# gchq/annchor

Hardware: AMD Instinct MI355X
Metric: knn_graph_builds_per_s (1 / Annchor.fit() wall-clock; BASELINE: k-NN graph build time + recall@k) (higher is better)
Workload: dtype int32 bit-vectors (Levenshtein) + f64 (bounds/regression/selection); 1 GPU; load_strings Levenshtein N=1600 n_anchors=15 k=25 p_work=0.12 niters=2; parallelism=one GPU

## Files before the change

annchor_amd/_native.py:

```python
import ctypes
import os

import numpy as np

_HERE = os.path.dirname(os.path.abspath(__file__))
LIB_PATH = os.environ.get("ANNCHOR_HIP_LIB", os.path.join(_HERE, "libannchor_hip.so"))

F_D, F_A, F_SID, F_IJS, F_I_PTR, F_I_IDX, F_FEATURES, F_NCM, F_RA, F_LABELS, F_THRESH, F_PROB, F_CAND, F_NEXT, F_DAD = range(1, 16)
_FIELD_DTYPE = {
    F_D: np.float64, F_A: np.int64, F_SID: np.uint64, F_IJS: np.int64, F_I_PTR: np.int64, F_I_IDX: np.int64,
    F_FEATURES: np.float64, F_NCM: np.uint8, F_RA: np.float64, F_LABELS: np.int64, F_THRESH: np.float64,
    F_PROB: np.float64, F_CAND: np.int64, F_NEXT: np.int64, F_DAD: np.float64,
}

METRIC_LEVENSHTEIN, METRIC_EUCLIDEAN_F32, METRIC_EUCLIDEAN_F64, METRIC_WASSERSTEIN = 1, 2, 3, 4
METRIC_COSINE_F32, METRIC_COSINE_F64 = 5, 6

_vp, _i32, _i64, _dbl = ctypes.c_void_p, ctypes.c_int32, ctypes.c_int64, ctypes.c_double
_SIGNATURES = {
    "annchor_create": (ctypes.c_int, [ctypes.c_int, ctypes.POINTER(_vp)]),
    "annchor_destroy": (None, [_vp]),
    "annchor_release_parked": (ctypes.c_int, []),
    "annchor_parked_bytes": (ctypes.c_int, [ctypes.c_int, ctypes.POINTER(_i64)]),
    "annchor_last_error": (ctypes.c_char_p, [_vp]),
# ... 7 lines not shown
    "annchor_set_strings": (ctypes.c_int, [_vp, _vp, _vp, _vp, _i64, _i32]),
    "annchor_set_strings_u16": (ctypes.c_int, [_vp, _vp, _vp, _vp, _i64, _i32]),
    "annchor_set_points_f32": (ctypes.c_int, [_vp, _vp, _i64, _i32]),
    "annchor_set_points_f64": (ctypes.c_int, [_vp, _vp, _i64, _i32]),
    "annchor_set_points_cosine_f32": (ctypes.c_int, [_vp, _vp, _i64, _i32]),
    "annchor_set_points_cosine_f64": (ctypes.c_int, [_vp, _vp, _i64, _i32]),
    "annchor_set_histograms": (ctypes.c_int, [_vp, _vp, _i64, _i32, _vp]),
    "annchor_set_opaque": (ctypes.c_int, [_vp, _i64]),
    "annchor_metric_pairs": (ctypes.c_int, [_vp, _vp, _i64, _vp]),
    "annchor_brute_force": (ctypes.c_int, [_vp, _i32, _vp, _vp]),
    "annchor_pick_anchors_maxmin": (ctypes.c_int, [_vp, _i32, _i64]),
    "annchor_pick_anchors_selected": (ctypes.c_int, [_vp, _vp, _i32]),
    "annchor_set_anchor_distances": (ctypes.c_int, [_vp, _vp, _i32, _vp, _i32]),
    "annchor_build_locality": (ctypes.c_int, [_vp, _i32, _i32, _i32, ctypes.POINTER(_i64), ctypes.POINTER(_i64)]),
    "annchor_build_query_locality": (ctypes.c_int, [_vp, _i64, _i32, _i32, ctypes.POINTER(_i64), ctypes.POINTER(_i64)]),
    "annchor_compute_features": (ctypes.c_int, [_vp]),
    "annchor_count_uncomputed": (ctypes.c_int, [_vp, ctypes.POINTER(_i64)]),
    "annchor_kth_uncomputed_dad": (ctypes.c_int, [_vp, _vp, _i32, _vp]),
    "annchor_bin_counts": (ctypes.c_int, [_vp, _vp, _i32, _vp]),
    "annchor_sampler_stats": (ctypes.c_int, [_vp, _vp, _i32, _vp, _vp, _vp, _vp]),
    "annchor_select_by_rank": (ctypes.c_int, [_vp, _vp, _i32, _vp, _vp, _i64, _vp]),
    "annchor_sample_pairs": (ctypes.c_int, [_vp, _vp, _i32, _vp, _vp, _vp, _i64, _vp, _vp, _vp]),
    "annchor_sample_pairs_device": (ctypes.c_int, [_vp, _vp, _i32, _vp, _vp, _vp, _i64]),
    "annchor_hash_sample_pairs_device": (ctypes.c_int, [_vp, _vp, _i32, _vp, _vp, ctypes.c_uint64, _vp]),
    "annchor_download_samples": (ctypes.c_int, [_vp, _vp, _vp, _vp, _vp]),
    "annchor_fit_regression_device": (ctypes.c_int, [_vp, _vp, _i32, _i32, _i32]),
    "annchor_fit_errors_device": (ctypes.c_int, [_vp]),
    "annchor_model_download": (ctypes.c_int, [_vp, _vp, _vp, _vp, _vp, _vp]),
    "annchor_errors_download": (ctypes.c_int, [_vp, _vp, _i64]),
    "annchor_model_download_with_errors": (ctypes.c_int, [_vp, _vp, _vp, _vp, _vp, _vp, _vp, _i64, ctypes.POINTER(_i64)]),
    "annchor_sample_pairs_device_draw": (ctypes.c_int, [_vp, _vp, _i32, _vp, _vp, ctypes.c_uint32, ctypes.POINTER(_i64), ctypes.POINTER(_i32)]),
    "annchor_legacy_choice_ranks_device": (ctypes.c_int, [_vp, ctypes.c_uint32, _vp, _vp, _i32, _vp, ctypes.POINTER(_i32)]),
    "annchor_hash_sample": (ctypes.c_int, [_vp, _vp, _i32, _vp, _vp, ctypes.c_uint64, _vp, ctypes.POINTER(_i64)]),
    "annchor_hash_sample_pairs": (ctypes.c_int, [_vp, _vp, _i32, _vp, _vp, ctypes.c_uint64, _vp, _vp, _vp, ctypes.POINTER(_i64)]),
    "annchor_legacy_prefetch": (ctypes.c_int, [ctypes.c_uint32, _i64]),
    "annchor_legacy_generate": (ctypes.c_int, [ctypes.c_uint32, _i64]),
    "annchor_legacy_generate_at_next_wait": (ctypes.c_int, [_vp, ctypes.c_uint32, _i64, _i64]),
    "annchor_legacy_choice_ranks": (ctypes.c_int, [ctypes.c_uint32, _vp, _vp, _i32, _vp, _vp]),
    "annchor_legacy_choice_begin": (ctypes.c_int, [ctypes.c_uint32, _vp, _vp, _i32, ctypes.POINTER(_vp)]),
    "annchor_legacy_choice_end": (ctypes.c_int, [_vp, _vp, _vp]),
    "annchor_ols_bins": (ctypes.c_int, [_vp, _vp, _vp, _i64, _i32, _vp, _i32, _vp, _vp, _vp, _vp]),
    "annchor_gather_features": (ctypes.c_int, [_vp, _vp, _i64, _vp]),
    "annchor_evaluate_samples": (ctypes.c_int, [_vp, _vp, _i64, _vp]),
    "annchor_set_samples": (ctypes.c_int, [_vp, _vp, _i64, _vp]),
    "annchor_predict_merge": (ctypes.c_int, [_vp, _vp, _i32, _vp, _vp, _i32, _i32, _vp]),
    "annchor_merge_host_prediction": (ctypes.c_int, [_vp, _vp, _i32, _i32]),
    "annchor_set_labels": (ctypes.c_int, [_vp, _vp]),
    "annchor_select_candidates": (ctypes.c_int, [_vp, _i32, _i32, _vp, _vp, _i32, _i64, _i32,
                                                 ctypes.POINTER(_i64), ctypes.POINTER(_i64)]),
    "annchor_select_prepare": (ctypes.c_int, [_vp, _i32, _i32]),
    "annchor_mark_candidates": (ctypes.c_int, [_vp]),
    "annchor_refine_candidates": (ctypes.c_int, [_vp]),
    "annchor_park_refine": (ctypes.c_int, [_vp, _i32]),
    "annchor_set_refined": (ctypes.c_int, [_vp, _vp, _i64]),
    "annchor_update_bounds": (ctypes.c_int, [_vp]),
    "annchor_neighbor_graph": (ctypes.c_int, [_vp, _i32, _vp, _vp]),
    "annchor_stream_bind": (ctypes.c_int, [_vp, _vp, _i64, _i32, _i64, _i32]),
    "annchor_stream_anchor_round": (ctypes.c_int, [_vp, _vp, _i32, _i32, ctypes.POINTER(_dbl), ctypes.POINTER(_i64)]),
    "annchor_stream_get_row": (ctypes.c_int, [_vp, _i64, _vp]),
    "annchor_stream_order": (ctypes.c_int, [_vp, _i32] + [ctypes.POINTER(_vp)] * 6 + [ctypes.POINTER(_i64), ctypes.POINTER(_i32),
                                                                                   ctypes.POINTER(_i32)]),
    "annchor_stream_knn": (ctypes.c_int, [_vp, _vp, _vp, _vp, _vp, _vp, _vp, _i64, _i32, _i32, _i32, _i32, _i32, _i32, _dbl, _i32, _i32, _vp,
                                          _vp, _vp, ctypes.POINTER(_i64)]),
    "annchor_stream_knn_begin": (ctypes.c_int, [_vp, _vp, _vp, _vp, _vp, _vp, _vp, _i64, _i32, _i32, _i32, _i32, _i32, _i32, _i32,
                                                ctypes.POINTER(_vp), ctypes.POINTER(_i64)]),
    "annchor_stream_knn_join": (ctypes.c_int, [_vp, _vp, _i32, ctypes.POINTER(_vp), ctypes.POINTER(_i64)]),
    "annchor_stream_join_rev_begin": (ctypes.c_int, [_vp, _vp, ctypes.POINTER(_vp), ctypes.POINTER(_vp), ctypes.POINTER(_i64)]),
    "annchor_stream_order_begin": (ctypes.c_int, [_vp, _i32, _i32, _i32, ctypes.POINTER(_vp), ctypes.POINTER(_vp), ctypes.POINTER(_i64)]),
    "annchor_stream_order_end": (ctypes.c_int, [_vp] + [ctypes.POINTER(_vp)] * 6 + [ctypes.POINTER(_i64), ctypes.POINTER(_i32),
                                                                                       ctypes.POINTER(_i32)]),
    "annchor_stream_last_counts": (ctypes.c_int, [_vp, ctypes.POINTER(_i64), ctypes.POINTER(_i64)]),
    "annchor_stream_last_kernel": (ctypes.c_int, [_vp, ctypes.POINTER(ctypes.c_int32), ctypes.POINTER(_i64)]),
    "annchor_stream_last_tile_kernels": (ctypes.c_int, [_vp, ctypes.POINTER(ctypes.c_int32), ctypes.POINTER(ctypes.c_int32)]),
    "annchor_stream_budget": (ctypes.c_int, [_i32, _dbl, _i32, ctypes.POINTER(_i32), ctypes.POINTER(_i32), ctypes.POINTER(_i32)]),
    "annchor_stream_knn_end": (ctypes.c_int, [_vp, _vp, _vp, _vp, ctypes.POINTER(_i64)]),
    "annchor_stream_knn_run": (ctypes.c_int, [_vp, _vp, _vp, _vp, _vp, _vp, _vp, _i64, _i32, _i32, _i32, _i32, _i32, _i32, _dbl, _i32, _i32,
                                               ctypes.POINTER(_i64)]),
    "annchor_stream_knn_fetch": (ctypes.c_int, [_vp, _vp, _vp, _vp]),
    "annchor_stream_query": (ctypes.c_int, [_vp, _vp, _vp, _vp, _vp, _vp, _vp, _i64, _i32, _i32, _i32, _i32, _dbl, _vp, _vp,
                                            ctypes.POINTER(_i64)]),
    "annchor_stream_bind_f64": (ctypes.c_int, [_vp, _vp, _i64, _i32, _i64, _vp, _vp, ctypes.POINTER(_vp)]),
    "annchor_stream_rerank64": (ctypes.c_int, [_vp, _i32, _vp, _vp]),
    "annchor_stream_query64": (ctypes.c_int, [_vp, _vp, _vp, _vp, _vp, _vp, _vp, _i64, _i32, _i32, _i32, _i32, _i32, _dbl, _vp, _i64, _i64,
                                              _vp, _vp, ctypes.POINTER(_i64)]),
    "annchor_stream_last_rerank64": (ctypes.c_int, [_vp, ctypes.POINTER(_i64), ctypes.POINTER(ctypes.c_int32)]),
    "annchor_stream_order_classes": (ctypes.c_int, [_vp, _vp, _i32, _vp, ctypes.POINTER(_i64), ctypes.POINTER(_i32), ctypes.POINTER(_i32)]),
    "annchor_stream_enemies": (ctypes.c_int, [_vp, _i32, _dbl, _vp, _vp, ctypes.POINTER(_i64)]),
    "annchor_stream_join_tables": (ctypes.c_int, [_vp, _vp, _i32, _i32, _i32, _vp]),
    "annchor_stream_hip_stream": (ctypes.c_int, [_vp, ctypes.POINTER(_vp)]),
    "annchor_stream_anchor_begin": (ctypes.c_int, [_vp, _i32, _i64, _i32, ctypes.POINTER(_vp), ctypes.POINTER(_vp), ctypes.POINTER(_i64)]),
    "annchor_stream_anchor_step": (ctypes.c_int, [_vp, _vp, _i32, _i32]),
    "annchor_stream_anchor_end": (ctypes.c_int, [_vp, _vp, _vp]),
    "annchor_stream_rows_begin": (ctypes.c_int, [_vp, _i32, _vp, ctypes.POINTER(_vp), ctypes.POINTER(_vp), ctypes.POINTER(_i64)]),
    "annchor_stream_rows_end": (ctypes.c_int, [_vp, _i32, _vp]),
    "annchor_stream_anchor_dists_begin": (ctypes.c_int, [_vp, _i32, _vp, ctypes.POINTER(_vp), ctypes.POINTER(_vp), ctypes.POINTER(_i64)]),
    "annchor_stream_lists_all": (ctypes.c_int, [_vp, _i32, _i64, ctypes.POINTER(_vp)]),
    "annchor_stream_route_begin": (ctypes.c_int, [_vp, _i32, _vp, _vp, ctypes.POINTER(_vp), _vp, ctypes.POINTER(_i64), ctypes.POINTER(_i64)]),
    "annchor_stream_route_recv": (ctypes.c_int, [_vp, _i64, ctypes.POINTER(_vp)]),
    "annchor_comm_unique_id": (ctypes.c_int, [_vp]),
    "annchor_comm_init": (ctypes.c_int, [_vp, _vp, _i32, _i32]),
    "annchor_comm_destroy": (ctypes.c_int, [_vp]),
    "annchor_comm_set_timeout": (ctypes.c_int, [_vp, ctypes.c_double]),
    "annchor_comm_preflight": (ctypes.c_int, [_vp, ctypes.c_double]),
    "annchor_comm_init_side": (ctypes.c_int, [_vp, _vp]),
    "annchor_comm_allgather_begin": (ctypes.c_int, [_vp, _vp, _vp, _i64]),
    "annchor_comm_side_join": (ctypes.c_int, [_vp]),
# ... 491 lines not shown
        pos, y = _c(pos, np.int64), _c(y, np.float64)
        self._chk(self.lib.annchor_set_samples(self.h, _ptr(pos), len(pos), _ptr(y)))

    def predict_merge(self, bins, W, c, first, is_metric, n_samples):
        bins, W, c = _c(bins, np.float64), _c(W, np.float64), _c(c, np.float64)
        sp = np.zeros(n_samples, dtype=np.float64)
        self._chk(self.lib.annchor_predict_merge(self.h, _ptr(bins), len(bins) - 1, _ptr(W), _ptr(c), int(first),
                                                 int(is_metric), _ptr(sp)))
        return sp

    def n_pairs(self):
        return self.field_size(F_NCM)

    def merge_host_prediction(self, pred, first, is_metric):
        pred = _c(pred, np.float64).reshape(-1)
        if pred.shape[0] != self.n_pairs():
            raise ValueError("regression.predict returned %d values for %d candidate pairs" % (pred.shape[0], self.n_pairs()))
        self._chk(self.lib.annchor_merge_host_prediction(self.h, _ptr(pred), int(first), int(is_metric)))

    def set_labels(self, labels):
        labels = _c(labels, np.int64).reshape(-1)
        if labels.shape[0] != self.n_pairs():
            raise ValueError("error_predictor.predict returned %d labels for %d candidate pairs" % (labels.shape[0], self.n_pairs()))
        if labels.size and (labels.min() < 0 or labels.max() >= 255):
            raise ValueError("error labels must lie in 0..254 (got %d..%d)" % (labels.min(), labels.max()))
        self._chk(self.lib.annchor_set_labels(self.h, _ptr(labels)))

    def select_candidates(self, n_neighbors, nmin, errs_list, n_refine, lookahead, n_labels=None):
        nc, nn = _i64(), _i64()
        if errs_list is None:
            self._chk(self.lib.annchor_select_candidates(self.h, int(n_neighbors), int(nmin), None, None, int(n_labels), int(n_refine),
                                                         int(lookahead), ctypes.byref(nc), ctypes.byref(nn)))
            return nc.value, nn.value
        ptr = np.zeros(len(errs_list) + 1, dtype=np.int64)
        np.cumsum([len(e) for e in errs_list], out=ptr[1:])
        errs = _c(np.concatenate(errs_list) if len(errs_list) else np.zeros(0), np.float64)
        self._chk(self.lib.annchor_select_candidates(self.h, int(n_neighbors), int(nmin), _ptr(errs), _ptr(ptr),
                                                     len(errs_list), int(n_refine), int(lookahead),
                                                     ctypes.byref(nc), ctypes.byref(nn)))
        return nc.value, nn.value

    def select_prepare(self, n_neighbors, nmin):
        self._chk(self.lib.annchor_select_prepare(self.h, int(n_neighbors), int(nmin)))

    def mark_candidates(self):
        self._chk(self.lib.annchor_mark_candidates(self.h))

    def refine_candidates(self):
        self._chk(self.lib.annchor_refine_candidates(self.h))

    def park_refine(self, action):
        self._chk(self.lib.annchor_park_refine(self.h, int(action)))

    def set_refined(self, exact):
        exact = _c(exact, np.float64)
        self._chk(self.lib.annchor_set_refined(self.h, _ptr(exact), len(exact)))

    def update_bounds(self):
        self._chk(self.lib.annchor_update_bounds(self.h))

    def neighbor_graph(self, k):
        idx = np.zeros((self.nx, k), dtype=np.int64)
        dist = np.zeros((self.nx, k), dtype=np.float64)
        self._chk(self.lib.annchor_neighbor_graph(self.h, int(k), _ptr(idx), _ptr(dist)))
        return idx, dist

    def stream_bind(self, X, global_base=0, device_ptr=None, shape=None):
        if device_ptr is not None:
            n, d = shape
            self._chk(self.lib.annchor_stream_bind(self.h, device_ptr, int(n), int(d), int(global_base), 1))
        else:
            X = _c(X, np.float32)
            n, d = X.shape
            self._chk(self.lib.annchor_stream_bind(self.h, _ptr(X), n, d, int(global_base), 0))
        self.nx, self.metric = int(n), METRIC_EUCLIDEAN_F32
        self._stream_dim = int(d)

    def stream_bind_f64(self, X, global_base=0, centre=None):
        X = _c(X, np.float64)
        n, d = X.shape
        cin = _c(centre, np.float64) if centre is not None else None
        if cin is not None and cin.shape != (d,):
            raise ValueError("centre must be float64 [%d]" % d)
        cout, rows = np.empty(d, dtype=np.float64), _vp()
        self._chk(self.lib.annchor_stream_bind_f64(self.h, _ptr(X), n, d, int(global_base), _ptr(cin), _ptr(cout), ctypes.byref(rows)))
        self.nx, self.metric = int(n), METRIC_EUCLIDEAN_F32
        self._stream_dim = int(d)
        return cout, rows.value

    def stream_rerank64(self, k, n_local, out=None):
        if out is not None:
            idx, dist = out.take(n_local, k)
        else:
            idx = np.empty((int(n_local), int(k)), dtype=np.int64)
            dist = np.empty((int(n_local), int(k)), dtype=np.float64)
        self._chk(self.lib.annchor_stream_rerank64(self.h, int(k), _ptr(idx), _ptr(dist)))
        return idx, dist

    def stream_query64(self, cols, n_all, nt_all, n_anchors, dim_padded, nn, nn_search, p_work, rows64, n_data, data_base=0):
        idx = np.empty((self.nx, nn), dtype=np.int64)
        dist = np.empty((self.nx, nn), dtype=np.float64)
        ev = _i64()
        self._chk(self.lib.annchor_stream_query64(self.h, cols["Xs"], cols["rs"], cols["perm"], cols["lo"], cols["hi"], cols["mid"],
                                                  int(n_all), int(nt_all), int(n_anchors), int(dim_padded), int(nn), int(nn_search),
                                                  float(p_work), rows64, int(n_data), int(data_base), _ptr(idx), _ptr(dist), ctypes.byref(ev)))
        return idx, dist, ev.value
# ... 338 lines not shown
```

annchor_amd/annchor.py:

```python
import time
from collections import Counter

import os
import sys

import numpy as np

from . import _native
from .distances import DeviceMetric
from .error_predictors import SimpleStratifiedErrorRegression
from .pickers import MaxMinAnchorPicker
from .regressors import SimpleStratifiedLinearRegression
from .samplers import DeviceStratifiedSampler, NothingToSample, SimpleStratifiedSampler
from .utils import get_exact_ijs_, get_function_from_input, test_parallelisation

from .distances import euclidean as distances_euclidean
from .distances import cosine as distances_cosine

_DRAW_OVERLAP = {"worker": True, "defer": "defer"}[os.environ.get("ANNCHOR_DRAW", "defer")]
PAIRLIST_MAX_POINTS = 30000
PAIRLIST_HARD_MAX = None


PAIRLIST_BITMAP_MAX_POINTS = 400000
# ... 378 lines not shown
                return
            self._samples_on_device = False
            if self._device_metric:
                (self.sample_ixs, self.n_samples, self.sample_bins, self.sample_features,
                 self.sample_y) = self.sampler.finish_device(ticket, evaluate=True)
                self._invalidate("ncm")
                self.evals += self.sample_y.shape[0]
                return
            self.sample_ixs, self.n_samples, self.sample_bins = self.sampler.finish_device(ticket)
        else:
            self.sample_ixs, self.n_samples, self.sample_bins = self.sampler.sample(
                self.features, self.feature_names, self.n_samples, self.not_computed_mask, self.random_seed)
        self.sample_ixs = np.asarray(self.sample_ixs, dtype=np.int64)
        self.sample_features = eng.gather_features(self.sample_ixs)
        if self._device_metric:
            self.sample_y = eng.evaluate_samples(self.sample_ixs)
        else:
            self.sample_ijs = self.IJs[self.sample_ixs]
            self.sample_y = np.asarray(self.get_exact_ijs(self.f, self.X, self.sample_ijs), dtype=np.float64)
            eng.set_samples(self.sample_ixs, self.sample_y)
        self._invalidate("ncm")
        self.evals += self.sample_y.shape[0]

    def fit_predict_regression(self):
        self._pair_list_stage("fit_predict_regression")
        self._model_on_device = False
        if self.__dict__.get("_samples_on_device") and self._models_on_device():
            self._engine.fit_regression_device(self.sample_bins, self._first_merge, self.is_metric)
            self._model_on_device, self._predict_on_device, self._fused_labels = True, True, True
            self._first_merge = False
            self._invalidate("RA", "labels")
            return
        self.regression.fit(self.sample_features, self.feature_names, self.sample_y, sample_bins=self.sample_bins)
        model = self.regression.coefficients() if type(self.regression) is SimpleStratifiedLinearRegression else None
        self._fused_labels = False
        if model is not None:
            bins, W, c = model
            self.sample_predict = self._engine.predict_merge(bins, W, c, self._first_merge, self.is_metric,
                                                             len(self.sample_ixs))
            self._fused_labels = (type(self.error_predictor) is SimpleStratifiedErrorRegression
                                  and self.error_predictor.partition_feature_name == "double anchor distance"
                                  and np.array_equal(bins, self.sample_bins))
        else:
            pred = np.asarray(self.regression.predict(self.features, self.feature_names), dtype=np.float64)
            self.sample_predict = pred[self.sample_ixs]
            self._engine.merge_host_prediction(pred, self._first_merge, self.is_metric)
        self._first_merge = False
        self._invalidate("RA", "labels")

    def fit_predict_errors(self):
        self._pair_list_stage("fit_predict_errors")
        if self._pipelined and self._fit_it is not None:
            nn = self.n_neighbors
            self._engine.select_prepare(nn, 3 * nn // 2 if self._fit_it == 0 else 0)
        if self.__dict__.get("_model_on_device"):
            self._engine.fit_errors_device()
            self._invalidate("labels")
            if self._fit_it is not None and self.__dict__.get("_make_stream"):
                self._make_stream(self._fit_it + 1)
            return
        self.error_predictor.fit(self.sample_features, self.feature_names, self.sample_y - self.sample_predict,
                                 sample_bins=self.sample_bins)
        if not self._fused_labels:
            labels = self._label_slots(self.error_predictor.predict(self.features, self.feature_names))
            self._engine.set_labels(labels)
        self._invalidate("labels")

    def _label_slots(self, labels):
        labels = np.asarray(labels)
        keys = list(self.error_predictor.labels)
        if keys == list(range(len(keys))):
            return labels
        order = np.argsort(np.asarray(keys), kind="stable")
        sk = np.asarray(keys)[order]
        at = np.minimum(np.searchsorted(sk, labels), len(sk) - 1)
        if not np.array_equal(sk[at], labels):
            raise ValueError("error_predictor.predict returned a label that is not in error_predictor.labels")
        return order[at]

    def select_refine_candidate_pairs(self, w=0.5, it=0):
        self._pair_list_stage("select_refine_candidate_pairs")
        nn = self.n_neighbors
        n_refine = int((self.p_work * self.N - self.na - self.n_samples) * w) + 1
        n_refine = 0 if n_refine < 0 else n_refine
        nmin = 3 * nn // 2 if it == 0 else 0
        if self.__dict__.get("_model_on_device"):
            nb = len(self.sample_bins) - 1
            ncand, nnext = self._engine.select_candidates(nn, nmin, None, n_refine, self.lookahead, n_labels=nb)
            self._device_model_nb = nb
        else:
            labels = list(self.error_predictor.labels)
            errs = [np.asarray(self.error_predictor.errs[lab], dtype=np.float64) for lab in labels]
            if labels != list(range(len(labels))) and self._fused_labels:
                raise NotImplementedError("the fused label pass numbers the partitions 0..L-1; got labels %r" % (labels[:8],))
            ncand, nnext = self._engine.select_candidates(nn, nmin, errs, n_refine, self.lookahead)
        self.n_refine = n_refine
        self._invalidate("RA", "thresh", "cand", "next")
        if self._pipelined and self._device_metric and ncand and it < self.niters - 1 and self._sampler_on_device():
            self._engine.mark_candidates()
            self._engine.park_refine(1)
            try:
                self._sample_ticket = self.sampler.begin_device(self._engine, self.n_samples, self.random_seed, overlap=_DRAW_OVERLAP,
                                                                **({"device_trace": True} if self._models_on_device() else {}))
            finally:
                self._engine.park_refine(2)
        elif self._device_metric:
            self._engine.refine_candidates()
        elif ncand:
            mapback = self._engine.download(_native.F_CAND)
            exact = np.asarray(self.get_exact_ijs(self.f, self.X, self.IJs[mapback]), dtype=np.float64)
            self._engine.set_refined(exact)
        self.evals += ncand
        self._invalidate("RA", "ncm")

    def _adopt_device_model(self, nb):
        W, c, status, ep, flags, flat = self._engine.model_download_with_errors(nb, 2 * int(self.n_samples) + 16)
        if flags[0] == 3:
            raise _native.NativeError("sample step: the draw's trace kernel gave up waiting for the host's partner stream "
                                      "(ANNCHOR_DRAW_STREAM_TIMEOUT_MS; ANNCHOR_DRAW_STREAM=0 uploads the partners instead)")
        if flags[0] == 1:
            raise _native.NativeError("sample step: a (bin, rank) entry does not exist (stale counts?)")
        if flags[0] or flags[1] or flags[2] or status.any() or flat is None:
            self._device_model_refused = (status.copy(), flags.copy())
            return False
        reg = self.regression
        reg.n_partitions, reg.sample_bins, reg.coef_, reg.intercept_ = nb, self.sample_bins, W, c
        self._device_err_ptr = ep
        ep_ = self.error_predictor
        ep_.partition_bins, ep_.n_partitions, ep_.labels = self.sample_bins, nb, range(nb)
        ep_.errs = {b: flat[ep[b]:ep[b + 1]].copy() for b in range(nb)}
        return True

    @property
    def nextback(self):
        return self._view("next", lambda: self._engine.download(_native.F_NEXT))

    @property
    def mapback(self):
        return self._view("cand", lambda: self._engine.download(_native.F_CAND))

    def update_anchor_points(self, timeout=None, chunk_size=None):
        self._pair_list_stage("update_anchor_points")
        self._engine.update_bounds()
        self._invalidate("features")

    def get_ann(self):
        self._pair_list_stage("get_ann")
        self.neighbor_graph = self._engine.neighbor_graph(self.n_neighbors)

    def fit(self):
        if self._streamed is not None:
            st = self._streamed.fit()
            self.neighbor_graph = st.neighbor_graph
            if self._cosine_streamed:
                self.neighbor_graph = (st.neighbor_graph[0], st.neighbor_graph[1] ** 2 / 2.0)
            self._cache["A"] = st.A
            self.evals, self.timings = st.evals, st.timings
            return self
        origin = time.perf_counter()
        t = self.timings = {}
        legacy_rng = self._sampler_on_device() and type(self.sampler) is SimpleStratifiedSampler
        ndraws = self.N + self.N // 2 + 4096
        seed0 = self.random_seed + getattr(self.sampler, "loop_num", 0)

        def make_stream(it):
            if legacy_rng and it < self.niters:
                s = time.perf_counter()
                _native.legacy_generate(seed0 + it, ndraws)
                t["rng_stream"] = t.get("rng_stream", 0.0) + time.perf_counter() - s

        self._make_stream = make_stream

        def stage(name, fn, *a, **k):
            s = time.perf_counter()
            fn(*a, **k)
            t[name] = t.get(name, 0.0) + time.perf_counter() - s
            if self.verbose:
                print("%40s: %6.3f | %6.3f" % (name, time.perf_counter() - s, time.perf_counter() - origin))

        evals0, loop0, n_samples0 = self.evals, getattr(self.sampler, "loop_num", None), self.n_samples
        self._pipelined = True
        self._device_models_off = False
        try:
            try:
                return self._fit_stages(stage, make_stream, t, origin)
            except _DeviceModelRefused:
                self.evals, self.n_samples = evals0, n_samples0
                if loop0 is not None:
                    self.sampler.loop_num = loop0
                self._first_merge, self._sample_ticket, self._model_on_device = True, None, False
                t.clear()
                ols, self.ols = self.ols, "lapack"
                try:
                    return self._fit_stages(stage, make_stream, t, origin)
                finally:
                    self.ols = ols
        finally:
            self._pipelined, self._fit_it, self._sample_ticket = False, None, None
            self._make_stream = None

    def _fit_stages(self, stage, make_stream, t, origin):
        stage("get_anchors", self.get_anchors)
        legacy_rng = self._sampler_on_device() and type(self.sampler) is SimpleStratifiedSampler
        ndraws = self.N + self.N // 2 + 4096
        seed0 = self.random_seed + getattr(self.sampler, "loop_num", 0)
        fused = self._models_on_device()
        if self._anchors_on_device:
            if legacy_rng:
                self._engine.legacy_generate_at_next_wait(seed0, ndraws)
        elif legacy_rng:
            _native.legacy_prefetch(seed0, ndraws)
        stage("get_locality", self.get_locality)
        stage("get_features", self.get_features)
        niters = self.niters
        for it in range(niters):
            if legacy_rng and not fused and it + 1 < niters:
                _native.legacy_prefetch(seed0 + it + 1, ndraws)
            try:
                stage("get_sample", self.get_sample)
            except NothingToSample as err:
                if it == 0:
                    raise ValueError("Sampler raised NothingToSample on first iteration.") from err
                print("Warning: main loop terminated early with nothing " + "left to sample.")
                break
            stage("fit_predict_regression", self.fit_predict_regression)
            self._fit_it = it
            stage("fit_predict_errors", self.fit_predict_errors)
            self._fit_it = None
            stage("select_refine_candidate_pairs", self.select_refine_candidate_pairs, w=1 / niters, it=it)
            if it < niters - 1:
                stage("update_anchor_points", self.update_anchor_points)
        stage("get_ann", self.get_ann)
        if self.__dict__.get("_model_on_device") and not self._adopt_device_model(self._device_model_nb):
            raise _DeviceModelRefused()
        t["total"] = time.perf_counter() - origin
        return self

    def query(self, Q, nn=15, p_work=0.3, get_exact_query_ijs=None):
        if self._streamed is not None:
            qt = np.float64 if self._float64_streamed else np.float32
            Qs = np.asarray(Q, dtype=qt)
            if self._cosine_streamed:
                Qs = (Qs / np.linalg.norm(Qs.astype(np.float64), axis=1)[:, None]).astype(qt)
            idx, dist = self._streamed.query(Qs, nn=nn, p_work=p_work)
            return (idx, dist ** 2 / 2.0) if self._cosine_streamed else (idx, dist)
        if self.p_work > 1:
            print("Warning: p_work should not exceed 1.  Setting it to 1.")
            self.p_work = 1.0
        nq, nx = len(Q), self.nx
        na = self.n_anchors * nq
        nbf = nq * nx
        limit = ((nq * nn * 3) // 2 - 1 + na) / nbf
# ... 160 lines not shown
```

annchor_amd/csrc/common.h:

```cpp
#pragma once
#include <hip/hip_runtime.h>

#include <cstdint>
#include <cstdio>
#include <cstring>
#include <string>
#include <vector>
#include <chrono>

#include "../../include/annchor_hip.h"

#define ANN_WAVE 64

struct DevBuf {
    void *p = nullptr;
    size_t cap = 0;
    bool in_arena = false;
    template <typename T> T *as() const { return reinterpret_cast<T *>(p); }
};

struct ProfEntry {
    const char *name;
    double ms = 0;
    int64_t launches = 0;
// ... 62 lines not shown
    void *comm_watch = nullptr;

    int na = 0, nA = 0;
    DevBuf Dt;
    DevBuf A;
    DevBuf anchorRank;
    DevBuf runmin, redval, redidx;

    DevBuf sid, cA, thr;
    int sid_nw = 1;
    DevBuf sidl, sidm;
    int sid_L = 0;
    DevBuf Kbits, Kpref;
    DevBuf deg, low, rowstart;
    DevBuf Iptr, Iidx;
    int64_t n = 0;
    DevBuf ij;
    bool have_bitmap = false;
    DevBuf colT, colM;

    DevBuf lb, ub, dad, RA, prob;
    DevBuf anc, ncm, label;
    bool have_features = false, have_RA = false;
    int64_t n_unc = -1;
    int64_t n_unc_after_features = -1;

    DevBuf spos, sy;
    DevBuf draw_J, draw_next, draw_q1;
    DevBuf sfeat, spred;
    DevBuf model;
    DevBuf ols_scratch;
    std::vector<DevBuf *> own_allocs;
    int prof_group_entry = -1;
    bool model_fitted = false;
    bool errs_on_device = false;
    int model_nb = 0;
    DevBuf dev_flags;
    bool dev_flags_clean = false;
    bool gn_err_clean = false;
    bool state_prewarmed = false;
    DevBuf sstats;
    DevBuf hs_key, hs_pos, hs_misc;
    int64_t nsamp = 0;

    DevBuf thresh;
    DevBuf cand, next;
    int64_t ncand = 0, nnext = 0;
    bool cand_marked = false;
    DevBuf gl_val, gl_pos, gl_cnt, gl_ncomp, marked, markcount;
    DevBuf gn_state;
    bool sel_prepared = false;
    int sel_k = 0, sel_nmin = 0;
    bool gn_pending = false;
    int gn_round = 0, gn_L = 0;
    DevBuf sel_hist, sel_state, blk_cnt, blk_off;
    DevBuf sel_pass_state;
    DevBuf tie_lists, tie_hist;
    const void *tie_hist_clean = nullptr;
    DevBuf sel2, sel_bufA, sel_bufB, sel_seg;
    const void *sel2_clean = nullptr;
    DevBuf errs, errptr;
    DevBuf ecdf_index;
    DevBuf cptr, cidx, cval;
    DevBuf c16, cbnd;
    DevBuf tmp0, tmp1, tmp2, tmp3;
    DevBuf scan_tmp;

    DevBuf stage_in, stage_out;

    bool prof_on = false;
    int prof_mode = 0;
    std::vector<hipEvent_t> ev_pool;
    std::vector<ProfEntry> prof;
    std::vector<PendingEvent> pending;
    hipEvent_t call_a = nullptr, call_b = nullptr;
    bool call_timed = false;
    static constexpr int PIN_SLOTS = 8;
    static constexpr size_t PIN_SLOT_BYTES = 64 * 1024;
    static constexpr size_t PIN_DL_BYTES = 1024 * 1024;
    static constexpr size_t PIN_TAIL_BYTES = 64;
    unsigned char *pin = nullptr;
    hipEvent_t pin_ev[PIN_SLOTS] = {};
    bool pin_busy[PIN_SLOTS] = {};
    int pin_next = 0;
};

const char *ann_set_err(annchor_ctx *c, const char *fmt, ...);

#define ANN_CHECK_HIP(c, expr)                                                                  \
    do {                                                                                        \
        hipError_t _e = (expr);                                                                 \
        if (_e != hipSuccess) {                                                                 \
            ann_set_err((c), "%s:%d: %s failed: %s", __FILE__, __LINE__, #expr,                 \
                        hipGetErrorString(_e));                                                 \
            return ANNCHOR_EHIP;                                                                \
        }                                                                                       \
    } while (0)

#define ANN_TRY(expr)                \
    do {                             \
        int _r = (expr);             \
        if (_r != ANNCHOR_OK) return _r; \
    } while (0)

#define ANN_REQUIRE(c, cond, code, ...)    \
    do {                                   \
        if (!(cond)) {                     \
// ... 37 lines not shown
    ProfScope(annchor_ctx *ctx, const char *name, double alg_bytes = 0);
    ~ProfScope();
};

static inline int ann_blocks(int64_t n, int per_block) { return (int)((n + per_block - 1) / per_block); }

__device__ __forceinline__ uint64_t ann_key_asc(double v)
{
    uint64_t u = (uint64_t)__double_as_longlong(v);
    return (u & 0x8000000000000000ull) ? ~u : (u | 0x8000000000000000ull);
}
__device__ __forceinline__ double ann_key_asc_inv(uint64_t k)
{
    uint64_t u = (k & 0x8000000000000000ull) ? (k & 0x7fffffffffffffffull) : ~k;
    return __longlong_as_double((long long)u);
}

template <typename T> __device__ __forceinline__ T ann_ldc(const T *__restrict__ p, int64_t t, int64_t n)
{
    return p[t < n ? t : n - 1];
}

#define ANN_STREAM_MIN_PAIRS (8ll << 20)
template <typename T> __device__ __forceinline__ void ann_store(T *p, T v, bool stream)
{
    if (stream) __builtin_nontemporal_store(v, p);
    else *p = v;
}
template <typename T> __device__ __forceinline__ T ann_load(const T *p, bool stream)
{
    return stream ? __builtin_nontemporal_load(p) : *p;
}

#define MAXBINS 64
struct RegModel {
    double e[MAXBINS + 1];
    double w[MAXBINS][3];
    double c[MAXBINS];
    int nb;
};
struct DeviceModel {
    RegModel reg;
    int32_t status[MAXBINS];
    int32_t err_status;
    int64_t rows[MAXBINS];
    int64_t errptr[MAXBINS + 1];
};

struct PairSource {
    const int2 *ij = nullptr;
    const int32_t *idx = nullptr;
    const int32_t *anchor = nullptr;
    int64_t n = 0;
    const double *pick_row = nullptr;
    double *pick_runmin = nullptr;
    int32_t *pick_out = nullptr;
    int pick_reset = 0;
    bool *pick_fused = nullptr;
};

#define ANN_MASK_ANCHORS 256
#define ANN_MAX_ANCHORS 1024
static_assert(ANN_MAX_ANCHORS < 0xffff, "wide sets list anchor ids as uint16, 0xffff pads");
static inline bool ann_sid_wide(int na) { return na > ANN_MASK_ANCHORS; }
__device__ __forceinline__ int sidm_common(const uint16_t *__restrict__ sidl, const uint64_t *__restrict__ sidm, int L, int na, int kw,
                                           int64_t i, int64_t w)
{
    const int lane = threadIdx.x & 63;
    int c = 0;
    for (int r = 0; r < L; ++r) {
        const int64_t e = i * L + r;
        const uint32_t pr = reinterpret_cast<const uint32_t *>(sidl)[e >> 1];
        const int a = __builtin_amdgcn_readfirstlane((int)((pr >> ((e & 1) * 16)) & 0xffffu));
        if (a >= na) continue;
        const uint64_t m = sidm[(size_t)a * kw + w];
        c += (int)((m >> lane) & 1ull);
    }
    return c;
}
template <int LC>
__device__ __forceinline__ int sidm_common_l(const uint16_t *__restrict__ sidl, const uint64_t *__restrict__ sidm, int na, int kw,
                                             int64_t i, int64_t w)
{
    const int lane = threadIdx.x & 63;
    int a[LC];
#pragma unroll
    for (int r = 0; r < LC; ++r) {
        const int64_t e = i * LC + r;
        const uint32_t pr = reinterpret_cast<const uint32_t *>(sidl)[e >> 1];
        a[r] = __builtin_amdgcn_readfirstlane((int)((pr >> ((e & 1) * 16)) & 0xffffu));
    }
    int c = 0;
#pragma unroll
    for (int r = 0; r < LC; ++r) {
        const uint64_t m = sidm[(size_t)(a[r] < na ? a[r] : 0) * kw + w];
        c += a[r] < na ? (int)((m >> lane) & 1ull) : 0;
    }
    return c;
}
template <int NW> struct Sid { uint64_t w[NW]; };
template <int NW> __device__ __forceinline__ Sid<NW> sid_ld(const uint64_t *__restrict__ sid, int64_t i)
{
    Sid<NW> s;
#pragma unroll
    for (int w = 0; w < NW; ++w) s.w[w] = sid[i * NW + w];
    return s;
// ... 46 lines not shown
```

annchor_amd/csrc/ctx.hip:

```cpp
#include <cstdarg>
#include <cstdlib>

#include "common.h"
#include <algorithm>
#include <chrono>
#include <mutex>

static std::string g_create_err;
void ann_stream_release(annchor_ctx *c);
void ann_enemies_release(annchor_ctx *c);
void ann_comm_release(annchor_ctx *c);
hipError_t ann_comm_guarded_sync(annchor_ctx *c, hipStream_t stream, const char *where);

const char *ann_set_err(annchor_ctx *c, const char *fmt, ...)
{
    char buf[1024];
    va_list ap;
    va_start(ap, fmt);
    vsnprintf(buf, sizeof buf, fmt, ap);
    va_end(ap);
    if (c && c->comm_aborted && c->err.rfind("collective timed out", 0) == 0) return c->err.c_str();
    if (c) c->err = buf; else g_create_err = buf;
    return c ? c->err.c_str() : g_create_err.c_str();
}
// ... 143 lines not shown
    Piece pieces[] = {{&c->dev_flags, sizeof(int32_t) * 16}, {&c->lev_cursors, 4 * sizeof(int32_t)}, {&c->sel_state, ann_sel_state_bytes()},
                      {&c->sel2, ann_sel2_table_bytes()},    {&c->tie_hist, ann_tie_hist_bytes()},   {&c->lev_ap, slot_bytes}};
    size_t need = 0;
    for (auto &q : pieces) {
        if (q.b->p) return ANNCHOR_OK;
        need += (q.bytes + 255) & ~(size_t)255;
    }
    if (c->arena_off + need > c->arena_size) return ANNCHOR_OK;
    char *first = c->arena + c->arena_off;
    for (auto &q : pieces) ANN_TRY(ann_reserve(c, *q.b, q.bytes));
    ANN_CHECK_HIP(c, hipMemsetAsync(first, 0, need, c->stream));
    c->dev_flags_clean = true;
    c->lev_cursor_epoch = 0;
    c->gn_err_clean = true;
    c->sel2_clean = c->sel2.p;
    c->tie_hist_clean = c->tie_hist.p;
    c->lev_ap_epoch = 0;
    c->state_prewarmed = true;
    return ANNCHOR_OK;
}

int ann_h2d(annchor_ctx *c, void *dst, const void *src, size_t bytes)
{
    if (bytes == 0) return ANNCHOR_OK;
    if (c->pin && bytes <= annchor_ctx::PIN_SLOT_BYTES) {
        const int sl = c->pin_next;
        c->pin_next = (sl + 1) % annchor_ctx::PIN_SLOTS;
        if (c->pin_busy[sl]) ANN_CHECK_HIP(c, hipEventSynchronize(c->pin_ev[sl]));
        unsigned char *slot = c->pin + (size_t)sl * annchor_ctx::PIN_SLOT_BYTES;
        memcpy(slot, src, bytes);
        ANN_CHECK_HIP(c, hipMemcpyAsync(dst, slot, bytes, hipMemcpyHostToDevice, c->stream));
        ANN_CHECK_HIP(c, hipEventRecord(c->pin_ev[sl], c->stream));
        c->pin_busy[sl] = true;
        return ANNCHOR_OK;
    }
    ANN_CHECK_HIP(c, hipMemcpyAsync(dst, src, bytes, hipMemcpyHostToDevice, c->stream));
    ANN_CHECK_HIP(c, ann_sync(c, __func__));
    return ANNCHOR_OK;
}

hipError_t ann_sync(annchor_ctx *c, const char *where)
{
    static const bool trace = getenv("ANNCHOR_SYNC_TRACE") != nullptr;
    static const bool timing = getenv("ANNCHOR_SYNC_TIMING") != nullptr;
    if (trace) fprintf(stderr, "sync %s\n", where);
    const long long t_in = timing ? ann_now_ns() : 0;
    if (c->idle_gen_n > c->idle_gen_done) {
        c->idle_gen_done = std::min(c->idle_gen_n, c->idle_gen_done + c->idle_gen_chunk);
        (void)ann_legacy_generate_upto(c->idle_gen_seed, c->idle_gen_n, c->idle_gen_done);
    }
    const long long t_w = timing ? ann_now_ns() : 0;
    const hipError_t rc = c->comm ? ann_comm_guarded_sync(c, c->stream, where) : hipStreamSynchronize(c->stream);
    if (timing) fprintf(stderr, "T wait %s %lld %lld %lld\n", where, t_in, t_w, ann_now_ns());
    if (c->lev_ap_probe_epoch) ann_lev_ap_probe(c);
    return rc;
}

extern "C" int annchor_legacy_generate_at_next_wait(annchor_ctx *c, uint32_t seed, int64_t ndraws, int64_t chunk)
{
    if (!c || ndraws < 0) return ANNCHOR_EINVAL;
    c->idle_gen_seed = seed;
    c->idle_gen_n = ndraws;
    c->idle_gen_done = 0;
    c->idle_gen_chunk = chunk > 0 ? chunk : ndraws;
    return ANNCHOR_OK;
}

int ann_d2h(annchor_ctx *c, void *dst, const void *src, size_t bytes)
{
    if (bytes == 0) return ANNCHOR_OK;
    if (c->pin && bytes <= annchor_ctx::PIN_DL_BYTES) {
        unsigned char *slot = c->pin + (size_t)annchor_ctx::PIN_SLOTS * annchor_ctx::PIN_SLOT_BYTES;
        ANN_CHECK_HIP(c, hipMemcpyAsync(slot, src, bytes, hipMemcpyDeviceToHost, c->stream));
        ANN_CHECK_HIP(c, ann_sync(c, __func__));
        memcpy(dst, slot, bytes);
        return ANNCHOR_OK;
    }
    ANN_CHECK_HIP(c, hipMemcpyAsync(dst, src, bytes, hipMemcpyDeviceToHost, c->stream));
    ANN_CHECK_HIP(c, ann_sync(c, __func__));
    return ANNCHOR_OK;
}

int ann_d2h2(annchor_ctx *c, void *dst1, const void *src1, size_t bytes1, void *dst2, const void *src2, size_t bytes2)
{
    const size_t off2 = (bytes1 + 63) & ~(size_t)63;
    if (c->pin && off2 + bytes2 <= annchor_ctx::PIN_DL_BYTES) {
        unsigned char *slot = c->pin + (size_t)annchor_ctx::PIN_SLOTS * annchor_ctx::PIN_SLOT_BYTES;
        ANN_CHECK_HIP(c, hipMemcpyAsync(slot, src1, bytes1, hipMemcpyDeviceToHost, c->stream));
        ANN_CHECK_HIP(c, hipMemcpyAsync(slot + off2, src2, bytes2, hipMemcpyDeviceToHost, c->stream));
        ANN_CHECK_HIP(c, ann_sync(c, __func__));
        memcpy(dst1, slot, bytes1);
        memcpy(dst2, slot + off2, bytes2);
        return ANNCHOR_OK;
    }
    ANN_TRY(ann_d2h(c, dst1, src1, bytes1));
    return ann_d2h(c, dst2, src2, bytes2);
}

int ann_d2h_then(annchor_ctx *c, void *dst, const void *src, size_t bytes, int (*then)(annchor_ctx *))
{
    if (!c->pin || bytes > annchor_ctx::PIN_DL_BYTES) {
        ANN_TRY(ann_d2h(c, dst, src, bytes));
        return then(c);
    }
    if (!c->dl_ev) ANN_CHECK_HIP(c, hipEventCreate(&c->dl_ev));
    unsigned char *slot = c->pin + (size_t)annchor_ctx::PIN_SLOTS * annchor_ctx::PIN_SLOT_BYTES;
    ANN_CHECK_HIP(c, hipMemcpyAsync(slot, src, bytes, hipMemcpyDeviceToHost, c->stream));
    ANN_CHECK_HIP(c, hipEventRecord(c->dl_ev, c->stream));
    const int rc = then(c);
    static const bool trace = getenv("ANNCHOR_SYNC_TRACE") != nullptr;
    static const bool timing = getenv("ANNCHOR_SYNC_TIMING") != nullptr;
    if (trace) fprintf(stderr, "sync %s\n", __func__);
    const long long t_w = timing ? ann_now_ns() : 0;
    ANN_CHECK_HIP(c, hipEventSynchronize(c->dl_ev));
    if (timing) fprintf(stderr, "T wait %s %lld %lld %lld\n", __func__, t_w, t_w, ann_now_ns());
    memcpy(dst, slot, bytes);
    return rc;
}

int ann_prof_entry(annchor_ctx *c, const char *name)
{
    for (size_t i = 0; i < c->prof.size(); ++i)
        if (c->prof[i].name == name || strcmp(c->prof[i].name, name) == 0) return (int)i;
    ProfEntry e;
    e.name = name;
    c->prof.push_back(e);
    return (int)c->prof.size() - 1;
}

static void prof_drain(annchor_ctx *c)
{
    for (auto &p : c->pending) {
        float ms = 0;
        if (hipEventSynchronize(p.b) == hipSuccess && hipEventElapsedTime(&ms, p.a, p.b) == hipSuccess)
            c->prof[p.entry].ms += ms;
        c->ev_pool.push_back(p.a);
        c->ev_pool.push_back(p.b);
    }
    c->pending.clear();
}

ProfScope::ProfScope(annchor_ctx *ctx, const char *name, double alg_bytes) : c(ctx)
{
    if (!c->prof_on) return;
    if (c->prof_mode == 2) {
        const size_t n = strlen(name);
        if (n < 6 || strcmp(name + n - 6, "_pairs") != 0) return;
    }
    entry = ann_prof_entry(c, name);
    c->prof[entry].launches += 1;
    c->prof[entry].alg_bytes += alg_bytes;
    if (entry == c->prof_group_entry) { entry = -1; return; }
    auto get = [&](hipEvent_t *e) {
        if (!c->ev_pool.empty()) { *e = c->ev_pool.back(); c->ev_pool.pop_back(); return true; }
        return hipEventCreate(e) == hipSuccess;
    };
    if (!get(&a) || !get(&b)) { entry = -1; return; }
    (void)hipEventRecord(a, c->stream);
}

ProfGroup::ProfGroup(annchor_ctx *ctx, const char *name) : c(ctx)
{
    if (!c->prof_on || c->prof_group_entry >= 0) return;
    if (c->prof_mode == 2) {
        const size_t n = strlen(name);
        if (n < 6 || strcmp(name + n - 6, "_pairs") != 0) return;
    }
// ... 542 lines not shown
```

annchor_amd/csrc/lev.hip:

```cpp
#include <cstdlib>

#include "common.h"
#include <atomic>
#include <type_traits>

#define LEV_THREADS 256
#define LEV_WAVES (LEV_THREADS / ANN_WAVE)

__device__ __forceinline__ uint32_t dpp_wave_shr1(uint32_t v)
{
    return (uint32_t)__builtin_amdgcn_update_dpp((int)v, (int)v, 0x138 , 0xf, 0xf, false);
}

struct LevArgs {
    const uint8_t *sym;
    const int32_t *soff;
    const int32_t *slen;
    const int2 *ij;
    const int32_t *idx;
    const int32_t *anchor;
    int64_t n;
    double *out;
    double *RA;
    uint8_t *ncm;
    int G;
    int P;
    int alphabet;
    int text_stride;
    int pm_bytes;
    int wave_bytes;
};

__device__ __forceinline__ void wave_lds_fence()
{
    __builtin_amdgcn_fence(__ATOMIC_RELEASE, "workgroup");
    __builtin_amdgcn_wave_barrier();
    __builtin_amdgcn_fence(__ATOMIC_ACQUIRE, "workgroup");
}

struct LevArgsR {
    LevArgs b;
    int GL;
    int pm_stride;
    const double *pick_row;
    double *pick_runmin;
    int32_t *pick_out;
    int pick_reset, pick_nx;
    const int32_t *perm;
    const int32_t *n0;
    int GL0, P0;
};

#define LEVR_PAD 64

template <int R> __global__ __launch_bounds__(ANN_WAVE) void k_lev_r(LevArgsR ar)
{
    extern __shared__ __attribute__((aligned(16))) unsigned char smem[];
    const LevArgs &a = ar.b;
    const int lane = threadIdx.x;
    const int GL = ar.GL, P = a.P, A = a.alphabet, PS = ar.pm_stride;
    const int g = lane / GL;
    const int w = lane - g * GL;
    const bool slot_ok = g < P;
    uint32_t *pm_g = reinterpret_cast<uint32_t *>(smem) + (size_t)(slot_ok ? g : 0) * A * PS;
    uint16_t *txt_g = reinterpret_cast<uint16_t *>(smem + a.pm_bytes + (size_t)(slot_ok ? g : 0) * a.text_stride);
    int *ssum = reinterpret_cast<int *>(smem + a.pm_bytes + (size_t)P * a.text_stride);
    const int64_t n_tasks = (a.n + P - 1) / P;
    const uint32_t row_bytes = (uint32_t)PS * 4u;
    typedef uint32_t vecR __attribute__((ext_vector_type(R)));

    if (slot_ok)
        for (int e = w * 8; e < a.text_stride / 2; e += GL * 8) *reinterpret_cast<uint4 *>(txt_g + e) = make_uint4(0, 0, 0, 0);

    int picked = -1;
    if (ar.pick_row) {
        double bv = -INFINITY;
        int bi = 0x7fffffff;
        const int nx = ar.pick_nx;
        for (int j0 = 0; j0 < nx; j0 += 64 * 8) {
            double d[8], rm[8];
#pragma unroll
            for (int e = 0; e < 8; ++e) {
                const int j = min(j0 + e * 64 + lane, nx - 1);
                d[e] = ar.pick_row[j];
                rm[e] = ar.pick_reset ? 0.0 : ar.pick_runmin[j];
            }
#pragma unroll
            for (int e = 0; e < 8; ++e) {
                const int j = j0 + e * 64 + lane;
                if (j < nx) {
                    const double v = ar.pick_reset ? d[e] : fmin(rm[e], d[e]);
                    if (blockIdx.x == 0) ar.pick_runmin[j] = v;
                    argmax_combine(bv, bi, v, j);
                }
            }
        }
#pragma unroll
        for (int off = 32; off > 0; off >>= 1) {
            const double ov = __shfl_xor(bv, off);
            const int oi = __shfl_xor(bi, off);
            argmax_combine(bv, bi, ov, oi);
        }
        picked = bi;
// ... 93 lines not shown
                const uint32_t nvp = hns | ~(d0 | hps), nvn = hps & d0;
                vp[r] = valid ? nvp : vp[r];
                vn[r] = valid ? nvn : vn[r];
                hp_up = hp;
                hn_up = hn;
            }
            out_hp = hp_up;
            out_hn = hn_up;
            __builtin_amdgcn_sched_barrier(0);
            eq = eq_n;
            c1 = c2;
        };
        int k_lo = min(GL - 1, max_steps), k_hi = (active && m > 0) ? n : 0x7fffffff;
#pragma unroll
        for (int off = 32; off > 0; off >>= 1) k_hi = min(k_hi, __shfl_xor(k_hi, off));
        k_hi = max(k_lo, min(__builtin_amdgcn_readfirstlane(k_hi), max_steps));
        int k = 0;
        for (; k < k_lo; ++k) column(k, std::true_type());
        for (; k + 2 <= k_hi; k += 2) { column(k, std::false_type()); column(k + 1, std::false_type()); }
        for (; k < k_hi; ++k) column(k, std::false_type());
        for (; k < max_steps; ++k) column(k, std::true_type());
        if (active) {
            int part = 0;
#pragma unroll
            for (int r = 0; r < R; ++r) {
                const int wi = w * R + r;
                const uint32_t rows = wi < Wp - 1 ? 0xffffffffu : (wi == Wp - 1 ? (0xffffffffu >> (31 - ((m - 1) & 31))) : 0u);
                part += __popc(vp[r] & rows) - __popc(vn[r] & rows);
            }
            if (part) atomicAdd(&ssum[g], part);
        }
        wave_lds_fence();
        if (active && w == 0) {
            const double d = (double)(n + ssum[g]);
            if (a.out) a.out[t_pair] = d;
            if (a.RA) { a.RA[opos] = d; a.ncm[opos] = 0; }
        }
        wave_lds_fence();
    }
}

template <int R> static int launch_r(annchor_ctx *c, LevArgs a, int64_t npairs, const PairSource &src)
{
    const int W = (c->maxlen + 31) / 32 > 0 ? (c->maxlen + 31) / 32 : 1;
    LevArgsR ar;
    ar.GL = (W + R - 1) / R;
    ar.pm_stride = ar.GL * R;
    a.G = ar.GL;
    a.P = 64 / ar.GL;
    a.pm_bytes = (int)((((size_t)a.P * a.alphabet * ar.pm_stride * 4) + 15) & ~(size_t)15);
    a.text_stride = 2 * (2 * LEVR_PAD + ((c->maxlen + 15) & ~15) + 16);
    a.wave_bytes = a.pm_bytes + a.P * a.text_stride + 256;
    ar.b = a;
    ar.pick_row = nullptr; ar.pick_runmin = nullptr; ar.pick_out = nullptr; ar.pick_reset = 0; ar.pick_nx = 0;
    if (src.anchor && src.pick_fused && c->nx <= 8192) {
        *src.pick_fused = true;
        if (src.pick_row) {
            ar.pick_row = src.pick_row; ar.pick_runmin = src.pick_runmin; ar.pick_out = src.pick_out;
            ar.pick_reset = src.pick_reset; ar.pick_nx = (int)c->nx;
        }
    }
    const size_t lds = (size_t)a.wave_bytes;
    ANN_REQUIRE(c, lds <= 160 * 1024, ANNCHOR_ELIMIT, "alphabet %d x length %d needs %zu B of LDS (> 160 KiB)", c->alphabet,
                c->maxlen, lds);
    if (lds > 64 * 1024)
        ANN_CHECK_HIP(c, hipFuncSetAttribute((const void *)k_lev_r<R>, hipFuncAttributeMaxDynamicSharedMemorySize, (int)lds));
    int64_t blocks = (npairs + a.P - 1) / a.P;
    const int64_t max_blocks = (int64_t)c->prop.multiProcessorCount * 32;
    if (blocks > max_blocks) blocks = max_blocks;
    k_lev_r<R><<<(int)blocks, ANN_WAVE, lds, c->stream>>>(ar);
    ANN_CHECK_HIP(c, hipGetLastError());
    return ANNCHOR_OK;
}


__device__ __forceinline__ uint32_t dpp_shr1_or(uint32_t v, uint32_t m)
{
    return (uint32_t)__builtin_amdgcn_update_dpp(0, (int)v, 0x138, 0xf, 0xf, true) | m;
}
__device__ __forceinline__ uint32_t dpp_shr1_and(uint32_t v, uint32_t m)
{
    return (uint32_t)__builtin_amdgcn_update_dpp(0, (int)v, 0x138, 0xf, 0xf, true) & m;
}

#define LEVF_ROW 128

__global__ __launch_bounds__(ANN_WAVE) void k_lev_f(LevArgsR ar)
{
    extern __shared__ __attribute__((aligned(16))) unsigned char smem[];
    const LevArgs &a = ar.b;
    const int lane = threadIdx.x;
    const int A = a.alphabet;
    unsigned char *pm_col = smem + (size_t)(lane >> 5) * A * LEVF_ROW + (size_t)(lane & 31) * 4;
    const int Pmax = ar.perm ? ar.P0 : a.P;
    int *ssum = reinterpret_cast<int *>(smem + a.pm_bytes + (size_t)Pmax * a.text_stride);

    int picked = -1;
    if (ar.pick_row) {
        double bv = -INFINITY;
        int bi = 0x7fffffff;
        const int nx = ar.pick_nx;
        for (int j0 = 0; j0 < nx; j0 += 64 * 8) {
            double d[8], rm[8];
#pragma unroll
            for (int e = 0; e < 8; ++e) {
                const int j = min(j0 + e * 64 + lane, nx - 1);
                d[e] = ar.pick_row[j];
                rm[e] = ar.pick_reset ? 0.0 : ar.pick_runmin[j];
            }
#pragma unroll
            for (int e = 0; e < 8; ++e) {
                const int j = j0 + e * 64 + lane;
                if (j < nx) {
                    const double v = ar.pick_reset ? d[e] : fmin(rm[e], d[e]);
                    if (blockIdx.x == 0) ar.pick_runmin[j] = v;
                    argmax_combine(bv, bi, v, j);
                }
            }
        }
#pragma unroll
        for (int off = 32; off > 0; off >>= 1) {
            const double ov = __shfl_xor(bv, off);
            const int oi = __shfl_xor(bi, off);
            argmax_combine(bv, bi, ov, oi);
        }
        picked = bi;
        if (blockIdx.x == 0 && lane == 0) *ar.pick_out = bi;
    }
    const int64_t n_short = ar.perm ? (int64_t)*ar.n0 : 0;
  for (int cls = ar.perm ? 0 : 1; cls < 2; ++cls) {
    const int GL = cls == 0 ? ar.GL0 : ar.GL, P = cls == 0 ? ar.P0 : a.P;
    const int64_t n_cls = ar.perm ? (cls == 0 ? n_short : a.n - n_short) : a.n;
    const int g = lane / GL;
    const int w = lane - g * GL;
    const bool slot_ok = g < P;
    uint8_t *txt_g = smem + a.pm_bytes + (size_t)(slot_ok ? g : 0) * a.text_stride;
    const int64_t n_tasks = (n_cls + P - 1) / P;
    if (slot_ok)
        for (int e = w * 16; e < a.text_stride; e += GL * 16) *reinterpret_cast<uint4 *>(txt_g + e) = make_uint4(0, 0, 0, 0);
    uint32_t hp_or = w == 0 ? 0x80000000u : 0u;
    uint32_t hn_and = w == 0 ? 0u : 0xffffffffu;
    asm volatile("" : "+v"(hp_or), "+v"(hn_and));

// ... 54 lines not shown
            const uint32_t c2 = tp[k + 2];
            const uint32_t eq_n = *reinterpret_cast<const uint32_t *>(pm_col + c1 * LEVF_ROW);
            const uint32_t hp_up = dpp_shr1_or(out_hp, hp_or), hn_up = dpp_shr1_and(out_hn, hn_and);
            __builtin_amdgcn_sched_barrier(0);
            const bool valid = !decltype(checked)::value || (uint32_t)(k - w) < un;
            const uint32_t c = hn_up >> 31;
            const uint32_t x = eq | c;
            const uint32_t t = __builtin_amdgcn_bitop3_b32(c, eq, vp, 0xa8);
            const uint32_t sm = t + vp;
            const uint32_t d0p = __builtin_amdgcn_bitop3_b32(sm, vp, x, 0xbe);
            const uint32_t hp = __builtin_amdgcn_bitop3_b32(vn, d0p, vp, 0xf1);
            const uint32_t d0 = d0p | vn;
            const uint32_t hn = d0 & vp;
            const uint32_t hps = __builtin_amdgcn_alignbit(hp, hp_up, 31);
            const uint32_t hns = __builtin_amdgcn_alignbit(hn, hn_up, 31);
            const uint32_t nvp = __builtin_amdgcn_bitop3_b32(hns, d0, hps, 0xf1);
            const uint32_t nvn = hps & d0;
            vp = valid ? nvp : vp;
            vn = valid ? nvn : vn;
            out_hp = hp;
            out_hn = hn;
            __builtin_amdgcn_sched_barrier(0);
            eq = eq_n;
            c1 = c2;
        };
        int k_lo = min(GL - 1, max_steps), k_hi = (active && m > 0) ? n : 0x7fffffff;
#pragma unroll
        for (int off = 32; off > 0; off >>= 1) k_hi = min(k_hi, __shfl_xor(k_hi, off));
        k_hi = max(k_lo, min(__builtin_amdgcn_readfirstlane(k_hi), max_steps));
        int k = 0;
        for (; k < k_lo; ++k) column(k, std::true_type());
        for (; k + 2 <= k_hi; k += 2) { column(k, std::false_type()); column(k + 1, std::false_type()); }
        for (; k < k_hi; ++k) column(k, std::false_type());
        for (; k < max_steps; ++k) column(k, std::true_type());
        if (active) {
            const uint32_t rows = w < Wp - 1 ? 0xffffffffu : (w == Wp - 1 ? (0xffffffffu >> (31 - ((m - 1) & 31))) : 0u);
            const int part = __popc(vp & rows) - __popc(vn & rows);
            if (part) atomicAdd(&ssum[g], part);
        }
        wave_lds_fence();
        if (active && w == 0) {
            const double d = (double)(n + ssum[g]);
            if (a.out) a.out[t_pair] = d;
            if (a.RA) { a.RA[opos] = d; a.ncm[opos] = 0; }
        }
        wave_lds_fence();
    }
  }
}

__global__ __launch_bounds__(256) void k_lev_classify(const int2 *__restrict__ ij, const int32_t *__restrict__ idx,
                                                      const int32_t *__restrict__ slen, int64_t n, int gl0,
                                                      int32_t *__restrict__ perm, int32_t *__restrict__ cursors,
                                                      int32_t *__restrict__ next_cursors)
{
    if (blockIdx.x == 0 && threadIdx.x < 2) next_cursors[threadIdx.x] = 0;
    __shared__ int wcnt[2][4];
    __shared__ int base[2];
    const int lane = threadIdx.x & 63, wave = threadIdx.x >> 6;
    const int64_t t = (int64_t)blockIdx.x * 256 + threadIdx.x;
    bool is_short = false, is_long = false;
    if (t < n) {
        const int2 p = ij[idx ? idx[t] : t];
        const int m = min(slen[p.x], slen[p.y]);
        is_short = ((m + 31) >> 5) <= gl0;
        is_long = !is_short;
    }
    const unsigned long long bs = __ballot(is_short), bl = __ballot(is_long);
    if (lane == 0) { wcnt[0][wave] = __popcll(bs); wcnt[1][wave] = __popcll(bl); }
    __syncthreads();
    if (threadIdx.x < 2) {
        const int tot = wcnt[threadIdx.x][0] + wcnt[threadIdx.x][1] + wcnt[threadIdx.x][2] + wcnt[threadIdx.x][3];
        base[threadIdx.x] = tot ? atomicAdd(&cursors[threadIdx.x], tot) : 0;
    }
    __syncthreads();
    const unsigned long long below = (1ull << lane) - 1ull;
    if (is_short) {
        int r = base[0] + __popcll(bs & below);
        for (int q = 0; q < wave; ++q) r += wcnt[0][q];
        perm[r] = (int32_t)t;
    } else if (is_long) {
        int r = base[1] + __popcll(bl & below);
        for (int q = 0; q < wave; ++q) r += wcnt[1][q];
        perm[n - 1 - r] = (int32_t)t;
    }
}

static int lev_next_cursors(annchor_ctx *c, int32_t **cur, int32_t **nxt)
{
    if (!c->lev_cursors.p) {
        ANN_TRY(ann_reserve(c, c->lev_cursors, 4 * sizeof(int32_t)));
        ANN_CHECK_HIP(c, hipMemsetAsync(c->lev_cursors.p, 0, 4 * sizeof(int32_t), c->stream));
        c->lev_cursor_epoch = 0;
    }
    *cur = c->lev_cursors.as<int32_t>() + 2 * (c->lev_cursor_epoch & 1);
    *nxt = c->lev_cursors.as<int32_t>() + 2 * ((c->lev_cursor_epoch + 1) & 1);
    ++c->lev_cursor_epoch;
    return ANNCHOR_OK;
}

static int launch_f(annchor_ctx *c, LevArgs a, int64_t npairs, const PairSource &src)
{
    const int W = (c->maxlen + 31) / 32 > 0 ? (c->maxlen + 31) / 32 : 1;
    LevArgsR ar;
    ar.GL = W;
    ar.pm_stride = 32;
    a.G = ar.GL;
    a.P = 64 / ar.GL;
    a.pm_bytes = 2 * a.alphabet * LEVF_ROW;
    a.text_stride = 2 * LEVR_PAD + ((c->maxlen + 15) & ~15) + 16;
    ar.perm = nullptr; ar.n0 = nullptr; ar.GL0 = 0; ar.P0 = 0;
    static const int cls_min = getenv("ANNCHOR_LEV_CLASS_MIN") ? atoi(getenv("ANNCHOR_LEV_CLASS_MIN")) : 4096;
    if (!src.anchor && c->lev_gl0 > 0 && npairs >= cls_min && npairs < (1ll << 31)) {
        const double fp = 1.0 - (1.0 - c->lev_frac0) * (1.0 - c->lev_frac0);
        const int P0 = 64 / c->lev_gl0;
        const double cost = fp * (double)a.P / (double)P0 + (1.0 - fp);
        if (cost < 0.93) {
            ANN_TRY(ann_reserve(c, c->lev_perm, sizeof(int32_t) * ((size_t)npairs + 4)));
            int32_t *perm = c->lev_perm.as<int32_t>();
            int32_t *cursors = nullptr, *next_cursors = nullptr;
            ANN_TRY(lev_next_cursors(c, &cursors, &next_cursors));
            k_lev_classify<<<ann_blocks(npairs, 256), 256, 0, c->stream>>>(src.ij, src.idx, a.slen, npairs, c->lev_gl0, perm,
                                                                           cursors, next_cursors);
            ar.perm = perm; ar.n0 = cursors; ar.GL0 = c->lev_gl0; ar.P0 = P0;
        }
    }
    a.wave_bytes = a.pm_bytes + (ar.perm ? ar.P0 : a.P) * a.text_stride + 256;
    ar.b = a;
    ar.pick_row = nullptr; ar.pick_runmin = nullptr; ar.pick_out = nullptr; ar.pick_reset = 0; ar.pick_nx = 0;
    if (src.anchor && src.pick_fused && c->nx <= 8192) {
        *src.pick_fused = true;
        if (src.pick_row) {
            ar.pick_row = src.pick_row; ar.pick_runmin = src.pick_runmin; ar.pick_out = src.pick_out;
            ar.pick_reset = src.pick_reset; ar.pick_nx = (int)c->nx;
        }
    }
    const size_t lds = (size_t)a.wave_bytes;
    ANN_REQUIRE(c, lds <= 160 * 1024, ANNCHOR_ELIMIT, "alphabet %d x length %d needs %zu B of LDS (> 160 KiB)", c->alphabet,
                c->maxlen, lds);
    if (lds > 64 * 1024)
        ANN_CHECK_HIP(c, hipFuncSetAttribute((const void *)k_lev_f, hipFuncAttributeMaxDynamicSharedMemorySize, (int)lds));
    int64_t blocks = (npairs + a.P - 1) / a.P;
    const int64_t max_blocks = (int64_t)c->prop.multiProcessorCount * 32;
    if (blocks > max_blocks) blocks = max_blocks;
    k_lev_f<<<(int)blocks, ANN_WAVE, lds, c->stream>>>(ar);
    ANN_CHECK_HIP(c, hipGetLastError());
    return ANNCHOR_OK;
}

struct LevArgsA {
    const uint8_t *sym;
    const int32_t *soff;
    const int32_t *slen;
    const int32_t *anchor;
    int64_t n;
    double *out;
    int alphabet, text_stride, pm_bytes, fb_stride;
    const double *pick_row;
    double *pick_runmin;
    int32_t *pick_out;
    int pick_reset, pick_nx;
};

struct LevArgsA2 {
    LevArgsA a;
    const int32_t *order;
    int n_short;
    int buf_stride;
    int pad;
};

__global__ __launch_bounds__(ANN_WAVE) void k_lev_a2(LevArgsA2 aa)
{
    extern __shared__ __attribute__((aligned(16))) unsigned char smem[];
    const LevArgsA &a = aa.a;
    const int lane = threadIdx.x, A = a.alphabet;
    const int ws = (aa.n_short + 1) >> 1;
    const bool packed = (int)blockIdx.x < ws;
    const int GL = packed ? 16 : 32;
    const int slot = lane / GL, w = lane - slot * GL, pair = slot >> 1, half = slot & 1;
    const int LP = packed ? 32 : 64;
// ... 134 lines not shown
        out_hn = hn;
        __builtin_amdgcn_sched_barrier(0);
        eq = eq_n;
        c1 = c2;
    };
    int k = 0;
    for (; k < k_lo; ++k) column(k, std::true_type());
    for (; k + 2 <= k_hi; k += 2) { column(k, std::false_type()); column(k + 1, std::false_type()); }
    for (; k < k_hi; ++k) column(k, std::false_type());
    for (; k < max_steps; ++k) column(k, std::true_type());

    const uint32_t rows = !have ? 0u : (w < Wp - 1 ? 0xffffffffu : (w == Wp - 1 ? (0xffffffffu >> (31 - ((m - 1) & 31))) : 0u));
    const int part = __popc(vp & rows) - __popc(vn & rows);
    int incl = part;
#pragma unroll
    for (int off = 1; off < 32; off <<= 1) {
        const int o = __shfl_up(incl, off, 32);
        if (w >= off) incl += o;
    }
    int val = (int)un + incl - part;
    if (m == 0) val = half ? n - h : h;
    int16_t *fbp = FB + (size_t)(pair < 2 ? pair : 0) * 2 * a.fb_stride;
    int16_t *fb = fbp + (size_t)half * a.fb_stride;
    if (have && w == 0) fb[0] = (int16_t)val;
#pragma unroll
    for (int b = 0; b < 32; ++b) {
        val += (int)((vp >> b) & 1u) - (int)((vn >> b) & 1u);
        if ((rows >> b) & 1u) fb[w * 32 + b + 1] = (int16_t)val;
    }
    wave_lds_fence();
    int best = 0x7fffffff;
    const int lp = lane & (LP - 1);
    if (have)
        for (int i = lp; i <= m; i += LP) best = min(best, (int)fbp[i] + (int)fbp[a.fb_stride + m - i]);
#pragma unroll
    for (int off = 32; off > 0; off >>= 1)
        if (off < LP) best = min(best, __shfl_xor(best, off));
    if (have && lp == 0) a.out[tq[pair]] = (double)best;
}

struct LevArgsP2 {
    const uint8_t *sym;
    const int32_t *soff;
    const int32_t *slen;
    const int2 *ij;
    const int32_t *idx;
    const int32_t *perm;
    const int32_t *cursors;
    int64_t n;
    double *out;
    double *RA;
    uint8_t *ncm;
    int alphabet, pm_bytes, fb_stride, buf_stride, pad;
};

__global__ __launch_bounds__(ANN_WAVE) void k_lev_p2(LevArgsP2 aa)
{
    extern __shared__ __attribute__((aligned(16))) unsigned char smem[];
    const LevArgsP2 &a = aa;
    const int lane = threadIdx.x, A = a.alphabet;
    const int n_short = a.cursors[0], n_long = a.cursors[1];
    const int ws = (n_short + 1) >> 1;
    for (int task = blockIdx.x; task < ws + n_long; task += gridDim.x) {
    const bool packed = task < ws;
    const int GL = packed ? 16 : 32;
    const int slot = lane / GL, w = lane - slot * GL, pair = slot >> 1, half = slot & 1;
    const int LP = packed ? 32 : 64;
    unsigned char *pm_col = smem + (size_t)(lane >> 5) * A * LEVF_ROW + (size_t)(lane & 31) * 4;
    uint8_t *bufs = smem + a.pm_bytes;
    int16_t *FB = reinterpret_cast<int16_t *>(bufs + 4 * aa.buf_stride);
    for (int e = lane * 16; e < 4 * aa.buf_stride; e += 64 * 16) *reinterpret_cast<uint4 *>(bufs + e) = make_uint4(0, 0, 0, 0);
    uint32_t hp_or = w == 0 ? 0x80000000u : 0u;
    uint32_t hn_and = w == 0 ? 0u : 0xffffffffu;
    asm volatile("" : "+v"(hp_or), "+v"(hn_and));
    int tq[2] = {-1, -1};
    if (packed) {
        tq[0] = a.perm[2 * task];
        if (2 * task + 1 < n_short) tq[1] = a.perm[2 * task + 1];
    } else {
        tq[0] = a.perm[n_short + (task - ws)];
    }
    int si[2] = {0, 0}, sj[2] = {0, 0}, li[2] = {0, 0}, lj[2] = {0, 0};
    int64_t opos[2] = {0, 0};
#pragma unroll
    for (int q = 0; q < 2; ++q)
        if (tq[q] >= 0) {
            opos[q] = a.idx ? (int64_t)a.idx[tq[q]] : (int64_t)tq[q];
            const int2 pq = a.ij[opos[q]];
            si[q] = pq.x; sj[q] = pq.y;
        }
#pragma unroll
    for (int q = 0; q < 2; ++q)
        if (tq[q] >= 0) {
            li[q] = a.slen[si[q]]; lj[q] = a.slen[sj[q]];
            const uint8_t *s0 = a.sym + a.soff[si[q]], *s1 = a.sym + a.soff[sj[q]];
            for (int ch = lane; ch < ((li[q] + 15) >> 4); ch += 64)
                reinterpret_cast<uint4 *>(bufs + (2 * q) * aa.buf_stride + aa.pad)[ch] = reinterpret_cast<const uint4 *>(s0)[ch];
            for (int ch = lane; ch < ((lj[q] + 15) >> 4); ch += 64)
                reinterpret_cast<uint4 *>(bufs + (2 * q + 1) * aa.buf_stride + aa.pad)[ch] = reinterpret_cast<const uint4 *>(s1)[ch];
        }
    wave_lds_fence();
    const bool have = pair < 2 && tq[pair < 2 ? pair : 0] >= 0 && (packed || pair == 0);
    const int pq = pair < 2 ? pair : 0;
    const int l0 = have ? li[pq] : 0, l1 = have ? lj[pq] : 0;
    const bool first_is_pattern = packed ? (l0 <= l1) : (l0 > l1);
    const int m = have ? (first_is_pattern ? l0 : l1) : 0;
    const int n = have ? (first_is_pattern ? l1 : l0) : 0;
    const uint8_t *pat = bufs + (2 * pq + (first_is_pattern ? 0 : 1)) * aa.buf_stride + aa.pad;
    const uint8_t *txt = bufs + (2 * pq + (first_is_pattern ? 1 : 0)) * aa.buf_stride + aa.pad;
    const int Wp = (m + 31) >> 5;
    for (int c = 0; c < A; ++c) *reinterpret_cast<uint32_t *>(pm_col + (size_t)c * LEVF_ROW) = 0u;
    if (have && w < Wp) {
// ... 350 lines not shown
            bool collected = (int)blockIdx.x >= ngroups;
            int polls = 0;
            for (;;) {
                if (!collected) {
                    const unsigned long long v = __hip_atomic_load(sl + min((int)blockIdx.x * 64 + lane, a.ntasks - 1), __ATOMIC_RELAXED,
                                                                   __HIP_MEMORY_SCOPE_AGENT);
                    if (__all((uint32_t)(v >> 32) == tag)) {
                        uint32_t gm = (uint32_t)v;
#pragma unroll
                        for (int off = 32; off > 0; off >>= 1) gm = max(gm, (uint32_t)__shfl_xor((int)gm, off));
                        if (lane == 0)
                            __hip_atomic_store(pl + blockIdx.x, ((unsigned long long)tag << 32) | gm, __ATOMIC_RELAXED, __HIP_MEMORY_SCOPE_AGENT);
                        collected = true;
                    }
                }
                if (collected) {
                    const unsigned long long v = __hip_atomic_load(pl + min(lane, ngroups - 1), __ATOMIC_RELAXED, __HIP_MEMORY_SCOPE_AGENT);
                    mx = (uint32_t)v;
                    if (__all((uint32_t)(v >> 32) == tag)) break;
                }
                if ((++polls & 7) == 0 || a.timeout_ticks == 0) {
                    if (__hip_atomic_load(a.abort_epoch, __ATOMIC_RELAXED, __HIP_MEMORY_SCOPE_AGENT) == a.epoch) return;
                    if (wall_clock64() - t0 > a.timeout_ticks) {
                        if (lane == 0) __hip_atomic_store(a.abort_epoch, a.epoch, __ATOMIC_RELAXED, __HIP_MEMORY_SCOPE_AGENT);
                        return;
                    }
                }
            }
#pragma unroll
            for (int off = 32; off > 0; off >>= 1) mx = max(mx, (uint32_t)__shfl_xor((int)mx, off));
            si = 0xffff - (int)(mx & 0xffffu);
            AP_STAMP(6);
        }
    }
    if (RESCUE) {
        __syncthreads();
        for (int j = threadIdx.x; j < nx; j += blockDim.x) a.rank[j] = -1;
        __syncthreads();
        if (threadIdx.x == 0)
            for (int r = 0; r < a.na; ++r) a.rank[s_A[r]] = r;
    } else {
        if (lane == 0) {
            a.rank[tq0] = rk0;
            if (tq1 >= 0) a.rank[tq1] = rk1;
        }
    }
}

static int launch_p2(annchor_ctx *c, const PairSource &src, double *d_out, double *d_RA, uint8_t *d_ncm)
{
    LevArgsP2 a;
    a.sym = c->sym.as<uint8_t>(); a.soff = c->soff.as<int32_t>(); a.slen = c->slen.as<int32_t>();
    a.ij = src.ij; a.idx = src.idx; a.n = src.n; a.out = d_out; a.RA = d_RA; a.ncm = d_ncm;
    a.alphabet = c->alphabet;
    a.pm_bytes = 2 * a.alphabet * LEVF_ROW;
    a.fb_stride = (c->maxlen + 2 + 7) & ~7;
    a.pad = ((c->maxlen / 2 + 48) + 15) & ~15;
    a.buf_stride = 2 * a.pad + ((c->maxlen + 15) & ~15) + 16;
    const size_t lds = (size_t)a.pm_bytes + 4 * (size_t)a.buf_stride + 4 * sizeof(int16_t) * a.fb_stride;
    ANN_REQUIRE(c, lds <= 160 * 1024, ANNCHOR_ELIMIT, "alphabet %d x length %d needs %zu B of LDS (> 160 KiB)", c->alphabet,
                c->maxlen, lds);
    ANN_TRY(ann_reserve(c, c->lev_perm, sizeof(int32_t) * (size_t)(src.n + 2)));
    int32_t *perm = c->lev_perm.as<int32_t>();
    int32_t *cursors = nullptr, *next_cursors = nullptr;
    ANN_TRY(lev_next_cursors(c, &cursors, &next_cursors));
    k_lev_classify<<<ann_blocks(src.n, 256), 256, 0, c->stream>>>(src.ij, src.idx, a.slen, src.n, 16, perm, cursors, next_cursors);
    a.perm = perm; a.cursors = cursors;
    if (lds > 64 * 1024)
        ANN_CHECK_HIP(c, hipFuncSetAttribute((const void *)k_lev_p2, hipFuncAttributeMaxDynamicSharedMemorySize, (int)lds));
    const int64_t L = c->nx - c->lev_nshort;
    const int64_t long_bound = std::min<int64_t>(src.n, L * (L + 1) / 2);
    const int64_t grid = std::min<int64_t>(src.n, (src.n + 1) / 2 + long_bound + 8);
    k_lev_p2<<<(int)grid, ANN_WAVE, lds, c->stream>>>(a);
    ANN_CHECK_HIP(c, hipGetLastError());
    return ANNCHOR_OK;
}

static int launch_a2(annchor_ctx *c, const PairSource &src, double *d_out)
{
    LevArgsA2 aa;
    LevArgsA &a = aa.a;
    a.sym = c->sym.as<uint8_t>(); a.soff = c->soff.as<int32_t>(); a.slen = c->slen.as<int32_t>();
    a.anchor = src.anchor; a.n = src.n; a.out = d_out; a.alphabet = c->alphabet;
    a.pm_bytes = 2 * a.alphabet * LEVF_ROW;
    a.text_stride = 2 * LEVR_PAD + ((c->maxlen + 15) & ~15) + 16;
    a.fb_stride = (c->maxlen + 2 + 7) & ~7;
    a.pick_row = nullptr; a.pick_runmin = nullptr; a.pick_out = nullptr; a.pick_reset = 0; a.pick_nx = 0;
    if (src.pick_fused && c->nx <= 8192) {
        *src.pick_fused = true;
        if (src.pick_row) {
            a.pick_row = src.pick_row; a.pick_runmin = src.pick_runmin; a.pick_out = src.pick_out;
            a.pick_reset = src.pick_reset; a.pick_nx = (int)c->nx;
        }
    }
    aa.order = c->lev_order.as<int32_t>();
    aa.n_short = c->lev_nshort;
    aa.pad = ((c->maxlen / 2 + 48) + 15) & ~15;
    aa.buf_stride = 2 * aa.pad + ((c->maxlen + 15) & ~15) + 16;
    size_t lds = (size_t)a.pm_bytes + 3 * (size_t)aa.buf_stride + 4 * sizeof(int16_t) * a.fb_stride;
    ANN_REQUIRE(c, lds <= 160 * 1024, ANNCHOR_ELIMIT, "alphabet %d x length %d needs %zu B of LDS (> 160 KiB)", c->alphabet,
                c->maxlen, lds);
    const int64_t blocks = (c->lev_nshort + 1) / 2 + (c->nx - c->lev_nshort);
    {
        const char *e = getenv("ANNCHOR_LEV_A2_LDS");
        const size_t want = e ? (size_t)atoll(e) : (size_t)40 * 1024;
        if (blocks <= (int64_t)c->prop.multiProcessorCount * 4 && want > lds && want <= 160 * 1024) lds = want;
    }
    if (lds > 64 * 1024)
        ANN_CHECK_HIP(c, hipFuncSetAttribute((const void *)k_lev_a2, hipFuncAttributeMaxDynamicSharedMemorySize, (int)lds));
    k_lev_a2<<<(int)blocks, ANN_WAVE, lds, c->stream>>>(aa);
    ANN_CHECK_HIP(c, hipGetLastError());
    return ANNCHOR_OK;
}

static std::atomic<int> g_lev_ap_strikes{0};
static std::atomic<int> g_lev_ap_off{0};
void ann_lev_ap_probe(annchor_ctx *c)
{
    const uint32_t epoch = c->lev_ap_probe_epoch;
// ... 211 lines not shown
            const uint32_t cin = hn_up >> 31;
            const uint32_t x = eq | cin;
            const uint32_t d0 = (((x & vp) + vp) ^ vp) | x | vn;
            const uint32_t hp = vn | ~(d0 | vp);
            const uint32_t hn = d0 & vp;
            const uint32_t hps = __builtin_amdgcn_alignbit(hp, hp_up, 31);
            const uint32_t hns = __builtin_amdgcn_alignbit(hn, hn_up, 31);
            const uint32_t nvp = hns | ~(d0 | hps), nvn = hps & d0;
            vp = valid ? nvp : vp;
            vn = valid ? nvn : vn;
            out_hp = hp;
            out_hn = hn;
        }
        if (active) {
            const uint32_t rows = w < Wp - 1 ? 0xffffffffu : (w == Wp - 1 ? (0xffffffffu >> (31 - ((m - 1) & 31))) : 0u);
            const int part = __popc(vp & rows) - __popc(vn & rows);
            if (part) atomicAdd(&ssum[g], part);
        }
        wave_lds_fence();
        if (active && w == 0) {
            const double d = (double)(n + ssum[g]);
            if (a.out) a.out[t_pair] = d;
            if (a.RA) { a.RA[opos] = d; a.ncm[opos] = 0; }
        }
        wave_lds_fence();
    }
}

static int launch_w(annchor_ctx *c, const PairSource &src, double *d_out, double *d_RA, uint8_t *d_ncm)
{
    LevArgsW a;
    a.sym = c->sym.as<uint16_t>(); a.soff = c->soff.as<int32_t>(); a.slen = c->slen.as<int32_t>();
    a.ij = src.ij; a.idx = src.idx; a.anchor = src.anchor; a.n = src.n; a.out = d_out; a.RA = d_RA; a.ncm = d_ncm;
    const int W = std::max(1, (c->maxlen + 31) / 32);
    ANN_REQUIRE(c, W <= 64, ANNCHOR_ELIMIT, "strings longer than 2048 symbols are not supported by this build (max %d)", c->maxlen);
    a.GL = W; a.P = 64 / W;
    a.text_stride = 2 * LEVR_PAD + ((c->maxlen + 7) & ~7) + 8;
    const size_t lds = (size_t)a.P * a.text_stride * 2 + 256;
    ANN_REQUIRE(c, lds <= 160 * 1024, ANNCHOR_ELIMIT, "strings of %d symbols need %zu B of LDS", c->maxlen, lds);
    if (lds > 64 * 1024)
        ANN_CHECK_HIP(c, hipFuncSetAttribute((const void *)k_lev_w, hipFuncAttributeMaxDynamicSharedMemorySize, (int)lds));
    int64_t blocks = (src.n + a.P - 1) / a.P;
    const int64_t max_blocks = (int64_t)c->prop.multiProcessorCount * 32;
    if (blocks > max_blocks) blocks = max_blocks;
    ProfScope ps(c, "levenshtein_pairs", (double)src.n * (4.0 * c->maxlen + 8));
    k_lev_w<<<(int)blocks, ANN_WAVE, lds, c->stream>>>(a);
    ANN_CHECK_HIP(c, hipGetLastError());
    return ANNCHOR_OK;
}

int ann_lev_launch(annchor_ctx *c, const PairSource &src, double *d_out, double *d_RA, uint8_t *d_ncm)
{
    if (src.n == 0) return ANNCHOR_OK;
    if (c->sym_wide) return launch_w(c, src, d_out, d_RA, d_ncm);
    LevArgs a;
    a.sym = c->sym.as<uint8_t>();
    a.soff = c->soff.as<int32_t>();
    a.slen = c->slen.as<int32_t>();
    a.ij = src.ij;
    a.idx = src.idx;
    a.anchor = src.anchor;
    a.n = src.n;
    a.out = d_out;
    a.RA = d_RA;
    a.ncm = d_ncm;
    int G = (c->maxlen + 31) / 32;
    if (G < 1) G = 1;
    ANN_REQUIRE(c, G <= 64, ANNCHOR_ELIMIT, "strings longer than 2048 symbols are not supported by this build (max %d)",
                c->maxlen);
    a.G = G;
    a.P = 64 / G;
    a.alphabet = c->alphabet;
    a.text_stride = ((c->maxlen + 15) & ~15) + 16;
    a.pm_bytes = (int)((((size_t)a.P * a.alphabet * G * 4) + 15) & ~(size_t)15);
    a.wave_bytes = a.pm_bytes + a.P * a.text_stride + 256;
    const char *env_r = getenv("ANNCHOR_LEV_R");
    {
        const int W = (c->maxlen + 31) / 32;
        const int R = env_r && atoi(env_r) == 1 ? 1 : 9;
        const char *env_a = getenv("ANNCHOR_LEV_ANCHOR");
        const bool anchor_split = !(env_a && atoi(env_a) == 0);
        if (src.anchor && d_out && !d_RA && R == 9 && W <= 32 && anchor_split && c->maxlen < 32000) {
            if (src.n == c->nx && c->lev_order.p) {
                ProfScope ps(c, "levenshtein_pairs", (double)src.n * (2.0 * c->maxlen + 8));
                return launch_a2(c, src, d_out);
            }
        }
        if (R == 9 && W <= 32) {
            ProfScope ps(c, "levenshtein_pairs", (double)src.n * (2.0 * c->maxlen + 8));
            const char *env_p = getenv("ANNCHOR_LEV_P2_MAX");
            const int pf = c->lev_gl0 > 0 ? std::max(1, 64 / c->lev_gl0) : a.P;
            const double cap = (double)c->prop.multiProcessorCount * 4.0 * pf;
            const bool p2 = env_p ? src.n <= atoll(env_p)
                                  : (pf <= 4 && ((double)src.n <= 0.37 * cap || ((double)src.n > cap && (double)src.n <= 1.83 * cap)));
            if (!src.anchor && src.ij && p2 && src.n >= 64 && c->maxlen < 32000) return launch_p2(c, src, d_out, d_RA, d_ncm);
            return launch_f(c, a, src.n, src);
        }
        ProfScope ps(c, "levenshtein_pairs", (double)src.n * (2.0 * c->maxlen + 8));
        return launch_r<1>(c, a, src.n, src);
    }
}
```

annchor_amd/csrc/select.hip:

```cpp
#include "common.h"
#include "rowsel.h"
#include "selstate.h"

__global__ __launch_bounds__(ROW_THREADS) void k_row_thresh(const int64_t *__restrict__ Iptr, RowSrc src, uint32_t k,
                                                           double *__restrict__ thresh, int cap)
{
    __shared__ RowSelShared sh;
    __shared__ RowCand rc;
    extern __shared__ __attribute__((aligned(16))) unsigned char dyn_rt[];
    uint64_t *keys = reinterpret_cast<uint64_t *>(dyn_rt);
    const int64_t i = row_of_block(gridDim.x);
    const int64_t b = Iptr[i];
    const int len = (int)(Iptr[i + 1] - b);
    if (len <= 0) { if (threadIdx.x == 0) thresh[i] = -INFINITY; return; }
    const RowView rv = row_view(src, i, b);
    const uint32_t kk = k >= (uint32_t)len ? (uint32_t)len - 1 : k;
    {
        const int cnt = row_candidates(rc, len, (int)kk + 1, [&](int s) { return ann_key_asc(rv.val(s)); }, [](int) { return true; },
                                       [](int, uint64_t, bool) {});
        const int cnts = cnt > (int)kk ? row_cand_shrink(rc, cnt, (int)kk + 1, src.shrink_min) : -1;
        if (cnts > (int)kk) {
            for (int e = threadIdx.x; e < cnts; e += ROW_THREADS) {
                const uint64_t ke = rc.key[e];
                uint32_t less = 0, leq = 0;
// ... 76 lines not shown
        if (kk < t) {
            const uint32_t o = atomicAdd(&cnt_lt, 1u);
            lkey[o] = kk; lslot[o] = s;
        }
    }
    __syncthreads();
    const uint32_t nlt = cnt_lt;
    uint32_t run = nlt;
    for (int base = 0; base < len && run < (uint32_t)want; base += ROW_THREADS) {
        const int s = base + threadIdx.x;
        const uint32_t f = (s < len && kf(s) == t) ? 1u : 0u;
        uint32_t tot;
        const uint32_t ex = row_block_scan(f, sh.wsum, &tot);
        if (f && run + ex < (uint32_t)want) { lkey[run + ex] = t; lslot[run + ex] = s; }
        run += tot;
        __syncthreads();
    }
    __syncthreads();
    for (int e = threadIdx.x; e < want; e += ROW_THREADS) {
        const uint64_t ke = lkey[e];
        const int32_t se = lslot[e];
        int r = 0;
        for (int o = 0; o < want; ++o) r += (lkey[o] < ke) || (lkey[o] == ke && lslot[o] < se);
        const int32_t p = Iidx[b + se];
        const int2 q = ij[p];
        gl_val[i * L + r] = ann_key_asc_inv(ke);
        gl_pos[i * L + r] = p;
        gl_oth[i * L + r] = q.x == (int)i ? q.y : q.x;
    }
}

__global__ void k_gn_twin(int64_t nx, int L, const int32_t *__restrict__ gl_pos, const int32_t *__restrict__ gl_oth,
                          const int32_t *__restrict__ gl_cnt, int32_t *__restrict__ gl_twin)
{
    const int64_t t = (int64_t)blockIdx.x * blockDim.x + threadIdx.x;
    if (t >= nx * L) return;
    const int64_t i = t / L;
    const int e = (int)(t - i * L);
    int tw = -1;
    if (e < gl_cnt[i]) {
        const int32_t p = gl_pos[t], j = gl_oth[t];
        const int cj = gl_cnt[j];
        for (int o = 0; o < cj; ++o)
            if (gl_pos[(int64_t)j * L + o] == p) { tw = o; break; }
    }
    gl_twin[t] = tw;
}

__global__ __launch_bounds__(256) void k_gn_round(int64_t nx, int nmin, int L, int Lw, const double *__restrict__ gl_val,
                                                 const int32_t *__restrict__ gl_oth, const int32_t *__restrict__ gl_twin,
                                                 const int32_t *__restrict__ gl_cnt, const int32_t *__restrict__ gl_ncomp,
                                                 const uint32_t *__restrict__ cur, uint32_t *__restrict__ nxt,
                                                 const int32_t *__restrict__ mout_cur, int32_t *__restrict__ mout_nxt,
                                                 int32_t *__restrict__ mout_clr, int32_t *__restrict__ changed, int32_t *__restrict__ err)
{
    const int lane = threadIdx.x & 63;
    const int64_t i = ((int64_t)blockIdx.x * blockDim.x + threadIdx.x) >> 6;
    if (i >= nx) return;
    if (lane == 0) mout_clr[i] = 0;
    const int cnt = gl_cnt[i], ncomp = gl_ncomp[i];
    const int ntodo = nmin - ncomp;
    const int chunks = (L + 63) / 64;
    bool active = !(ntodo <= 0 || (cnt == 0 && ncomp == 0));
    if (active && cnt <= ntodo && cnt < L) { if (lane == 0) *err = 1; active = false; }
    int m = active ? mout_cur[i] : 0;
    if (active)
        for (int ch = 0; ch < chunks; ++ch) {
            const int e = ch * 64 + lane;
            bool earlier = false;
            if (e < cnt) {
                const int32_t o = gl_oth[i * L + e], tw = gl_twin[i * L + e];
                earlier = o < i && tw >= 0 && ((cur[(int64_t)o * Lw + (tw >> 5)] >> (tw & 31)) & 1u);
            }
            m += __popcll(__ballot(earlier));
        }
    const int need = ntodo + 1 - m;
    double t = 0;
    bool found = false;
    if (active && need > 0) {
        int cum = 0;
        for (int ch = 0; ch < chunks && !found; ++ch) {
            const int e = ch * 64 + lane;
            bool um = false;
            double v = 0.0;
            if (e < cnt) {
                const int32_t o = gl_oth[i * L + e], tw = gl_twin[i * L + e];
                v = gl_val[i * L + e];
                um = !(o < i && tw >= 0 && ((cur[(int64_t)o * Lw + (tw >> 5)] >> (tw & 31)) & 1u));
            }
            const unsigned long long mb = __ballot(um);
            const int cm = __popcll(mb);
            if (cum + cm >= need) {
                const int want = need - cum - 1;
                const int myrank = __popcll(mb & ((1ull << lane) - 1ull));
                const unsigned long long hit = __ballot(um && myrank == want);
                t = __shfl(v, __ffsll((unsigned long long)hit) - 1);
                found = true;
            }
            cum += cm;
        }
        if (!found && lane == 0) *err = 2;
    }
    bool diff = false;
    for (int ch = 0; ch < chunks; ++ch) {
        const int e = ch * 64 + lane;
        bool mark = false;
        int32_t o = 0, tw = -1;
        if (found && e < cnt) {
            o = gl_oth[i * L + e]; tw = gl_twin[i * L + e];
            const bool earlier = o < i && tw >= 0 && ((cur[(int64_t)o * Lw + (tw >> 5)] >> (tw & 31)) & 1u);
            mark = !earlier && gl_val[i * L + e] < t;
        }
        const unsigned long long mb = __ballot(mark);
        const int w0 = 2 * ch, w1 = 2 * ch + 1;
        if (lane == 0) {
            if (w0 < Lw) { const uint32_t v0 = (uint32_t)mb; diff |= cur[i * Lw + w0] != v0; nxt[i * Lw + w0] = v0; }
            if (w1 < Lw) { const uint32_t v1 = (uint32_t)(mb >> 32); diff |= cur[i * Lw + w1] != v1; nxt[i * Lw + w1] = v1; }
        }
        if (mark && tw < 0 && o > i) atomicAdd(&mout_nxt[o], 1);
    }
    if (lane == 0 && diff) atomicOr(changed, 1);
}

__global__ void k_gn_apply(int64_t nx, int L, int Lw, const int32_t *__restrict__ gl_pos, const int32_t *__restrict__ gl_cnt,
                           const uint32_t *__restrict__ masks, double *__restrict__ RA)
{
    const int64_t t = (int64_t)blockIdx.x * blockDim.x + threadIdx.x;
    if (t >= nx * L) return;
    const int64_t i = t / L;
    const int e = (int)(t - i * L);
    if (e < gl_cnt[i] && ((masks[i * Lw + (e >> 5)] >> (e & 31)) & 1u)) RA[gl_pos[t]] = -1.0;
}

__global__ __launch_bounds__(64) void k_gn_sweep_lds(int64_t nx, int nmin, int L, const double *__restrict__ gl_val,
                                                    const int32_t *__restrict__ gl_pos, const int32_t *__restrict__ gl_oth,
                                                    const int32_t *__restrict__ gl_twin, const int32_t *__restrict__ gl_cnt,
                                                    const int32_t *__restrict__ gl_ncomp, double *__restrict__ RA,
                                                    int32_t *__restrict__ err)
{
    extern __shared__ __attribute__((aligned(16))) unsigned char dyn[];
    const int lane = threadIdx.x;
    const int Lw = (L + 31) / 32;
    uint32_t *mflag = reinterpret_cast<uint32_t *>(dyn);
    int32_t *mcount = reinterpret_cast<int32_t *>(mflag + (size_t)nx * Lw);
    for (int64_t t = lane; t < nx * Lw; t += 64) mflag[t] = 0;
    for (int64_t t = lane; t < nx; t += 64) mcount[t] = 0;
    __syncthreads();
    const int chunks = (L + 63) / 64;
    double nv = 0; int32_t np_ = 0, no = 0, nt = -1; int ncnt = 0, nncomp = 0;
    auto fetch = [&](int64_t r) {
        if (r < nx) {
            ncnt = gl_cnt[r]; nncomp = gl_ncomp[r];
            if (lane < L) { nv = gl_val[r * L + lane]; np_ = gl_pos[r * L + lane]; no = gl_oth[r * L + lane]; nt = gl_twin[r * L + lane]; }
        }
    };
    fetch(0);
    for (int64_t i = 0; i < nx; ++i) {
        const double v0 = nv; const int32_t p0 = np_, o0 = no, t0 = nt; const int cnt = ncnt, ncomp = nncomp;
        fetch(i + 1);
        const int ntodo = nmin - ncomp;
        if (ntodo <= 0 || (cnt == 0 && ncomp == 0)) continue;
        if (cnt <= ntodo && cnt < L) { if (lane == 0) *err = 1; continue; }
        const int need = ntodo + 1 - mcount[i];
        if (need <= 0) continue;
        double t = 0;
        bool found = false;
        int cum = 0;
        for (int ch = 0; ch < chunks && !found; ++ch) {
            const int e = ch * 64 + lane;
            const bool valid = e < cnt;
            const double v = ch == 0 ? v0 : (valid ? gl_val[i * L + e] : 0.0);
            const bool um = valid && !((mflag[i * Lw + (e >> 5)] >> (e & 31)) & 1u);
            const unsigned long long m = __ballot(um);
            const int cm = __popcll(m);
            if (cum + cm >= need) {
                const int want = need - cum - 1;
                const int myrank = __popcll(m & ((1ull << lane) - 1ull));
                const unsigned long long hit = __ballot(um && myrank == want);
                t = __shfl(v, __ffsll((unsigned long long)hit) - 1);
                found = true;
// ... 559 lines not shown
        flag[p] = prob[p] == t ? 1 : 0;
        scr[p] = (double)ann_tie_scramble(p);
    }
}

__device__ __forceinline__ int cut_class(double v, double t, unsigned long long rk, const double *RA, int64_t p)
{
    if (v > t) return 2;
    if (v != t) return 0;
    if (rk == ~0ull) return 2;
    const unsigned long long kk = ann_tie_scramble(p);
    return kk < rk ? 2 : (kk == rk ? 1 : 0);
}

__global__ __launch_bounds__(CP_THREADS) void k_cut_count(const double *__restrict__ prob, const double *__restrict__ RA, int64_t n,
                                                         const CutState *__restrict__ cs, uint32_t *__restrict__ blk, int nsub)
{
    __shared__ uint32_t acc[4];
    if (threadIdx.x < 4) acc[threadIdx.x] = 0;
    __syncthreads();
    const double t1 = cs->t1, t5 = cs->t5;
    const unsigned long long rk1 = cs->rk1, rk5 = cs->rk5;
    uint32_t g1 = 0, q1 = 0, g5 = 0, q5 = 0;
    for (int sub = 0; sub < nsub; ++sub) {
        const int64_t base = ((int64_t)blockIdx.x * nsub + sub) * CP_SUBTILE;
        if (base >= n) break;
        double v[CP_ITEMS];
#pragma unroll
        for (int k = 0; k < CP_ITEMS; ++k) v[k] = ann_ldc(prob, base + (int64_t)k * CP_THREADS + threadIdx.x, n);
#pragma unroll
        for (int k = 0; k < CP_ITEMS; ++k) {
            const int64_t p = base + (int64_t)k * CP_THREADS + threadIdx.x;
            if (p < n && v[k] >= 0.0) {
                const int c1 = cut_class(v[k], t1, rk1, RA, p), c5 = cut_class(v[k], t5, rk5, RA, p);
                g1 += c1 == 2; q1 += c1 == 1; g5 += c5 == 2; q5 += c5 == 1;
            }
        }
    }
    unsigned long long pk = (unsigned long long)g1 | ((unsigned long long)q1 << 16) | ((unsigned long long)g5 << 32) |
                            ((unsigned long long)q5 << 48);
#pragma unroll
    for (int off = 32; off > 0; off >>= 1) pk += __shfl_xor(pk, off);
    if ((threadIdx.x & 63) == 0) {
        atomicAdd(&acc[0], (uint32_t)(pk & 0xffff)); atomicAdd(&acc[1], (uint32_t)((pk >> 16) & 0xffff));
        atomicAdd(&acc[2], (uint32_t)((pk >> 32) & 0xffff)); atomicAdd(&acc[3], (uint32_t)(pk >> 48));
    }
    __syncthreads();
    if (threadIdx.x < 4) blk[(size_t)blockIdx.x * 4 + threadIdx.x] = acc[threadIdx.x];
}

#define CS_THREADS 1024
#define CS_ITEMS 4
__global__ __launch_bounds__(CS_THREADS) void k_cut_scan(const uint32_t *__restrict__ blk, int nb, CutState *__restrict__ cs,
                                                        int64_t *__restrict__ off)
{
    __shared__ unsigned long long wsum[CS_THREADS / 64];
    const int lane = threadIdx.x & 63, wave = threadIdx.x >> 6;
    auto block_scan = [&](unsigned long long v, unsigned long long *total) -> unsigned long long {
        unsigned long long inc = v;
#pragma unroll
        for (int o = 1; o < 64; o <<= 1) { unsigned long long x = __shfl_up(inc, o); if (lane >= o) inc += x; }
        __syncthreads();
        if (lane == 63) wsum[wave] = inc;
        __syncthreads();
        unsigned long long base = 0, tot = 0;
        for (int w = 0; w < CS_THREADS / 64; ++w) { const unsigned long long x = wsum[w]; if (w < wave) base += x; tot += x; }
        *total = tot;
        return base + inc - v;
    };
    const uint4 *blk4 = reinterpret_cast<const uint4 *>(blk);
    unsigned long long g = 0;
    for (int t0 = threadIdx.x; t0 < nb; t0 += CS_THREADS * CS_ITEMS) {
        uint4 b[CS_ITEMS];
#pragma unroll
        for (int e = 0; e < CS_ITEMS; ++e) b[e] = ann_ldc(blk4, t0 + e * CS_THREADS, nb);
#pragma unroll
        for (int e = 0; e < CS_ITEMS; ++e)
            if (t0 + e * CS_THREADS < nb) g += (unsigned long long)b[e].x | ((unsigned long long)b[e].z << 32);
    }
    unsigned long long T;
    block_scan(g, &T);
    const int64_t T1 = (int64_t)(T & 0xffffffffull), T5 = (int64_t)(T >> 32);
    const int64_t e1 = cs->all1 ? (1ll << 62) : cs->K1 - T1;
    const int64_t e5 = cs->all5 ? (1ll << 62) : cs->K5 - T5;
    const bool both_all = cs->all1 && cs->all5;
    unsigned long long c_eq = 0, c_out = 0;
    for (int base = 0; base < nb; base += CS_THREADS * CS_ITEMS) {
        const int t0 = base + threadIdx.x * CS_ITEMS;
        uint4 b[CS_ITEMS];
#pragma unroll
        for (int e = 0; e < CS_ITEMS; ++e) {
            b[e] = ann_ldc(blk4, t0 + e, nb);
            if (t0 + e >= nb) b[e] = make_uint4(0, 0, 0, 0);
        }
        unsigned long long eqs = 0;
#pragma unroll
        for (int e = 0; e < CS_ITEMS; ++e) eqs += (unsigned long long)b[e].y | ((unsigned long long)b[e].w << 32);
        unsigned long long tot;
        unsigned long long ex = c_eq + block_scan(eqs, &tot);
        c_eq += tot;
        int64_t p1[CS_ITEMS], p5[CS_ITEMS];
        unsigned long long outv[CS_ITEMS], outs = 0;
#pragma unroll
        for (int e = 0; e < CS_ITEMS; ++e) {
            p1[e] = (int64_t)(ex & 0xffffffffull);
            p5[e] = (int64_t)(ex >> 32);
            const int64_t eq1 = b[e].y, eq5 = b[e].w;
            const int64_t take1 = min(eq1, max((int64_t)0, e1 - p1[e]));
            const int64_t take5 = min(eq5, max((int64_t)0, e5 - p5[e]));
            const int64_t ncand = (int64_t)b[e].x + take1;
            const int64_t nbig = (int64_t)b[e].z + take5;
            const int64_t nnext = both_all ? nbig : nbig - ncand;
            outv[e] = (unsigned long long)ncand | ((unsigned long long)nnext << 32);
            outs += outv[e];
            ex += (unsigned long long)eq1 | ((unsigned long long)eq5 << 32);
        }
        unsigned long long exo = c_out + block_scan(outs, &tot);
        c_out += tot;
#pragma unroll
        for (int e = 0; e < CS_ITEMS; ++e) {
            if (t0 + e < nb) {
                int64_t *o = off + (size_t)(t0 + e) * 4;
                o[0] = p1[e]; o[1] = p5[e]; o[2] = (int64_t)(exo & 0xffffffffull); o[3] = (int64_t)(exo >> 32);
            }
            exo += outv[e];
        }
    }
    if (threadIdx.x == 0) { cs->e1 = e1; cs->e5 = e5; cs->ncand = (int64_t)(c_out & 0xffffffffull); cs->nnext = (int64_t)(c_out >> 32); }
}

__global__ __launch_bounds__(CP_THREADS) void k_cut_emit(const double *__restrict__ prob, const double *__restrict__ RA, int64_t n,
                                                        const CutState *__restrict__ cs, const int64_t *__restrict__ off,
                                                        int32_t *__restrict__ cand, int32_t *__restrict__ next, int nsub)
{
    __shared__ uint32_t wsum[CP_THREADS / 64];
    const double t1 = cs->t1, t5 = cs->t5;
    const unsigned long long rk1 = cs->rk1, rk5 = cs->rk5;
    const int64_t e1 = cs->e1, e5 = cs->e5;
    const bool both_all = cs->all1 && cs->all5;
    auto scan2 = [&](uint32_t a, uint32_t b, uint32_t *ea, uint32_t *eb, uint32_t *ta, uint32_t *tb) {
        uint32_t tot;
        const uint32_t packed = row_block_scan((a << 16) | b, wsum, &tot);
        __syncthreads();
        *ea = packed >> 16;
        *eb = packed & 0xffffu;
        *ta = tot >> 16;
        *tb = tot & 0xffffu;
    };
    int64_t R1 = off[(size_t)blockIdx.x * 4], R5 = off[(size_t)blockIdx.x * 4 + 1];
    int64_t WC = off[(size_t)blockIdx.x * 4 + 2], WN = off[(size_t)blockIdx.x * 4 + 3];
    for (int sub = 0; sub < nsub; ++sub) {
        const int64_t sbase = ((int64_t)blockIdx.x * nsub + sub) * CP_SUBTILE;
        if (sbase >= n) break;
        const int64_t base = sbase + (int64_t)threadIdx.x * CP_ITEMS;
        double v[CP_ITEMS];
        int8_t k1[CP_ITEMS], k5[CP_ITEMS];
        uint32_t q1 = 0, q5 = 0;
#pragma unroll
        for (int k = 0; k < CP_ITEMS; ++k) {
            v[k] = (base + k < n) ? prob[base + k] : -1.0;
            k1[k] = k5[k] = 0;
            if (v[k] >= 0.0) {
                k1[k] = (int8_t)cut_class(v[k], t1, rk1, RA, base + k);
                k5[k] = (int8_t)cut_class(v[k], t5, rk5, RA, base + k);
                q1 += k1[k] == 1; q5 += k5[k] == 1;
            }
        }
        uint32_t x1, x5, tq1, tq5;
        scan2(q1, q5, &x1, &x5, &tq1, &tq5);
        int64_t r1 = R1 + x1, r5 = R5 + x5;
        uint8_t fc[CP_ITEMS], fn[CP_ITEMS];
        uint32_t nc = 0, nn = 0;
#pragma unroll
        for (int k = 0; k < CP_ITEMS; ++k) {
            bool c1 = false, c5 = false;
            if (v[k] >= 0.0) {
                c1 = k1[k] == 2 || (k1[k] == 1 && r1 < e1);
                c5 = k5[k] == 2 || (k5[k] == 1 && r5 < e5);
                r1 += k1[k] == 1;
                r5 += k5[k] == 1;
            }
            fc[k] = c1;
            fn[k] = both_all ? c5 : (c5 && !c1);
            nc += fc[k];
            nn += fn[k];
        }
        uint32_t oc, on, tc, tn;
        scan2(nc, nn, &oc, &on, &tc, &tn);
        int64_t wc = WC + oc, wn = WN + on;
#pragma unroll
        for (int k = 0; k < CP_ITEMS; ++k) {
            if (fc[k]) cand[wc++] = (int32_t)(base + k);
            if (fn[k]) next[wn++] = (int32_t)(base + k);
        }
        R1 += tq1; R5 += tq5; WC += tc; WN += tn;
    }
}

#define SEL_ERR_OFF 256
#define SEL_STATE_BYTES (SEL_ERR_OFF + 256)
static_assert(sizeof(CutState) <= SEL_ERR_OFF, "the error flag sits behind the cut state");
static inline int32_t *gn_err_ptr(annchor_ctx *c) { return reinterpret_cast<int32_t *>(c->sel_state.as<char>() + SEL_ERR_OFF); }
size_t ann_sel_state_bytes() { return SEL_STATE_BYTES; }
#define GN_BATCH 8

static int select_stage_a(annchor_ctx *c, int32_t n_neighbors, int32_t nmin)
{
    const int64_t n = c->n, nx = c->nx;
    c->gn_pending = false;
    ANN_TRY(ann_reserve(c, c->thresh, sizeof(double) * (size_t)nx));
    ANN_CHECK_HIP(c, hipEventRecord(c->call_a, c->stream));
    RowSrc rsrc;
    ANN_TRY(ann_transpose_columns(c, &rsrc));
    {
        ProfScope ps(c, "row_kth_threshold", (double)n * 24.0);
        int cap = 2;
        if (!rsrc.T) ANN_TRY(row_pick_cap(c, k_row_thresh, nx, nx, 0, &cap));
        ANN_TRY(row_lds_prepare(c, k_row_thresh, (size_t)cap * 8));
        k_row_thresh<<<(int)nx, ROW_THREADS, (size_t)cap * 8, c->stream>>>(c->Iptr.as<int64_t>(), rsrc, (uint32_t)n_neighbors,
                                                                         c->thresh.as<double>(), cap);
    }
    if (nmin > 0) {
        const int L = nmin + 1;
        ANN_REQUIRE(c, L <= 1024, ANNCHOR_ELIMIT, "nmin=%d too large", nmin);
        ANN_TRY(ann_reserve(c, c->gl_val, sizeof(double) * (size_t)nx * L));
        ANN_TRY(ann_reserve(c, c->gl_pos, sizeof(int32_t) * (size_t)nx * L * 3));
        ANN_TRY(ann_reserve(c, c->gl_cnt, sizeof(int32_t) * (size_t)nx));
        ANN_TRY(ann_reserve(c, c->gl_ncomp, sizeof(int32_t) * (size_t)nx));
        ANN_TRY(ann_reserve(c, c->sel_state, SEL_STATE_BYTES));
        if (!c->gn_err_clean) {
            ANN_CHECK_HIP(c, hipMemsetAsync(gn_err_ptr(c), 0, 4, c->stream));
        }
        c->gn_err_clean = false;
        {
            ProfScope ps(c, "guarantee_nmin_lists", (double)n * 26.0);
            const size_t tail = (((size_t)L * 12) + 15) & ~(size_t)15;
            int cap = 2;
            if (!rsrc.T) ANN_TRY(row_pick_cap(c, k_gn_lists, nx, nx, tail, &cap));
            ANN_TRY(row_lds_prepare(c, k_gn_lists, (size_t)cap * 8 + tail));
            k_gn_lists<<<(int)nx, ROW_THREADS, (size_t)cap * 8 + tail, c->stream>>>(
                c->Iptr.as<int64_t>(), rsrc, c->ij.as<int2>(), L,
                c->gl_val.as<double>(), c->gl_pos.as<int32_t>(), c->gl_pos.as<int32_t>() + (size_t)nx * L,
                c->gl_cnt.as<int32_t>(), c->gl_ncomp.as<int32_t>(), cap);
        }
        const size_t sweep_lds = (size_t)nx * (((size_t)L + 31) / 32 * 4 + 4);
        const size_t ring_lds = sweep_lds + 2 * (size_t)GN_B * L * 20 + 64 * 20 + 4 * GN_B * 4 + 64 + 16;
        const char *gn_env = getenv("ANNCHOR_GN_SWEEP");
        if (!gn_env || strcmp(gn_env, "sequential") != 0) {
            ProfScope ps(c, "guarantee_nmin_sweep", (double)nx * L * 21.0);
            int32_t *oth = c->gl_pos.as<int32_t>() + (size_t)nx * L, *twin = oth + (size_t)nx * L;
            k_gn_twin<<<ann_blocks(nx * L, 256), 256, 0, c->stream>>>(nx, L, c->gl_pos.as<int32_t>(), oth,
                                                                     c->gl_cnt.as<int32_t>(), twin);
            const int Lw = (L + 31) / 32;
            const size_t mask_bytes = sizeof(uint32_t) * (size_t)nx * Lw, mout_bytes = sizeof(int32_t) * (size_t)nx;

            ANN_TRY(ann_reserve(c, c->gn_state, 2 * mask_bytes + 3 * mout_bytes + sizeof(int32_t) * GN_BATCH));
            uint32_t *masks[2] = {c->gn_state.as<uint32_t>(), c->gn_state.as<uint32_t>() + (size_t)nx * Lw};
            int32_t *mout[3];
            for (int q = 0; q < 3; ++q) mout[q] = reinterpret_cast<int32_t *>(c->gn_state.as<char>() + 2 * mask_bytes + q * mout_bytes);
            int32_t *changed = reinterpret_cast<int32_t *>(c->gn_state.as<char>() + 2 * mask_bytes + 3 * mout_bytes);
            ANN_CHECK_HIP(c, hipMemsetAsync(c->gn_state.p, 0, 2 * mask_bytes + 3 * mout_bytes + sizeof(int32_t) * GN_BATCH, c->stream));
            int round = 0;
            for (int q = 0; q < GN_BATCH; ++q, ++round)
                k_gn_round<<<ann_blocks(nx * 64, 256), 256, 0, c->stream>>>(
                    nx, nmin, L, Lw, c->gl_val.as<double>(), oth, twin, c->gl_cnt.as<int32_t>(), c->gl_ncomp.as<int32_t>(),
                    masks[round & 1], masks[(round + 1) & 1], mout[round % 3], mout[(round + 1) % 3], mout[(round + 2) % 3],
                    changed + q, gn_err_ptr(c));
            c->gn_pending = true; c->gn_round = round; c->gn_L = L;
        } else if (L <= GN_LMAX && ring_lds <= 156 * 1024) {
            ProfScope ps(c, "guarantee_nmin_sweep", (double)nx * L * 21.0);
            int32_t *oth = c->gl_pos.as<int32_t>() + (size_t)nx * L, *twin = oth + (size_t)nx * L;
            k_gn_twin<<<ann_blocks(nx * L, 256), 256, 0, c->stream>>>(nx, L, c->gl_pos.as<int32_t>(), oth,
                                                                     c->gl_cnt.as<int32_t>(), twin);
            ANN_CHECK_HIP(c, hipFuncSetAttribute((const void *)k_gn_sweep_ring, hipFuncAttributeMaxDynamicSharedMemorySize,
                                                 (int)ring_lds));
            k_gn_sweep_ring<<<1, 256, ring_lds, c->stream>>>(nx, nmin, L, c->gl_val.as<double>(), c->gl_pos.as<int32_t>(), oth, twin,
                                                            c->gl_cnt.as<int32_t>(), c->gl_ncomp.as<int32_t>(),
                                                            c->RA.as<double>(), gn_err_ptr(c));
        } else if (sweep_lds <= 150 * 1024) {
            ProfScope ps(c, "guarantee_nmin_sweep", (double)nx * L * 21.0);
            int32_t *oth = c->gl_pos.as<int32_t>() + (size_t)nx * L, *twin = oth + (size_t)nx * L;
            k_gn_twin<<<ann_blocks(nx * L, 256), 256, 0, c->stream>>>(nx, L, c->gl_pos.as<int32_t>(), oth,
                                                                     c->gl_cnt.as<int32_t>(), twin);
            if (sweep_lds > 64 * 1024)
                ANN_CHECK_HIP(c, hipFuncSetAttribute((const void *)k_gn_sweep_lds, hipFuncAttributeMaxDynamicSharedMemorySize,
                                                     (int)sweep_lds));
            k_gn_sweep_lds<<<1, 64, sweep_lds, c->stream>>>(nx, nmin, L, c->gl_val.as<double>(), c->gl_pos.as<int32_t>(), oth,
                                                           twin, c->gl_cnt.as<int32_t>(), c->gl_ncomp.as<int32_t>(),
                                                           c->RA.as<double>(), gn_err_ptr(c));
        } else {
            ANN_TRY(ann_reserve(c, c->marked, (size_t)n));
            ANN_TRY(ann_reserve(c, c->markcount, sizeof(int32_t) * (size_t)nx));
            ANN_CHECK_HIP(c, hipMemsetAsync(c->marked.p, 0, (size_t)n, c->stream));
            ANN_CHECK_HIP(c, hipMemsetAsync(c->markcount.p, 0, sizeof(int32_t) * (size_t)nx, c->stream));
            ProfScope ps(c, "guarantee_nmin_sweep", (double)nx * L * 13.0);
            k_gn_sequential<<<1, 64, 0, c->stream>>>(nx, nmin, L, c->gl_val.as<double>(), c->gl_pos.as<int32_t>(),
                                                    c->gl_cnt.as<int32_t>(), c->gl_ncomp.as<int32_t>(), c->ij.as<int2>(),
                                                    c->RA.as<double>(), c->marked.as<uint8_t>(), c->markcount.as<int32_t>(),
                                                    gn_err_ptr(c));
        }
    }
    return ANNCHOR_OK;
}

static int select_stage_finish(annchor_ctx *c)
{
    if (!c->gn_pending) return ANNCHOR_OK;
    const int64_t nx = c->nx;
    const int L = c->gn_L, Lw = (L + 31) / 32, nmin = L - 1;
    const size_t mask_bytes = sizeof(uint32_t) * (size_t)nx * Lw, mout_bytes = sizeof(int32_t) * (size_t)nx;
    uint32_t *masks[2] = {c->gn_state.as<uint32_t>(), c->gn_state.as<uint32_t>() + (size_t)nx * Lw};
    int32_t *mout[3];
    for (int q = 0; q < 3; ++q) mout[q] = reinterpret_cast<int32_t *>(c->gn_state.as<char>() + 2 * mask_bytes + q * mout_bytes);
    int32_t *changed = reinterpret_cast<int32_t *>(c->gn_state.as<char>() + 2 * mask_bytes + 3 * mout_bytes);
    int32_t *oth = c->gl_pos.as<int32_t>() + (size_t)nx * L, *twin = oth + (size_t)nx * L;
    int round = c->gn_round;
    for (;;) {
        int32_t h_changed[GN_BATCH];
        ANN_TRY(ann_d2h(c, h_changed, changed, sizeof h_changed));
        if (h_changed[GN_BATCH - 1] == 0) break;
        ANN_REQUIRE(c, round <= (int)nx + GN_BATCH, ANNCHOR_EHIP, "guarantee_nmin rounds did not settle");
        ANN_CHECK_HIP(c, hipMemsetAsync(changed, 0, sizeof(int32_t) * GN_BATCH, c->stream));
        for (int q = 0; q < GN_BATCH; ++q, ++round)
            k_gn_round<<<ann_blocks(nx * 64, 256), 256, 0, c->stream>>>(
                nx, nmin, L, Lw, c->gl_val.as<double>(), oth, twin, c->gl_cnt.as<int32_t>(), c->gl_ncomp.as<int32_t>(),
                masks[round & 1], masks[(round + 1) & 1], mout[round % 3], mout[(round + 1) % 3], mout[(round + 2) % 3],
                changed + q, gn_err_ptr(c));
    }
    k_gn_apply<<<ann_blocks(nx * L, 256), 256, 0, c->stream>>>(nx, L, Lw, c->gl_pos.as<int32_t>(), c->gl_cnt.as<int32_t>(),
                                                              masks[round & 1], c->RA.as<double>());
    ANN_CHECK_HIP(c, hipGetLastError());
    c->gn_pending = false;
    return ANNCHOR_OK;
}

size_t ann_tie_hist_bytes() { return sizeof(uint32_t) * 2 * TIE_BINS; }

extern "C" int annchor_select_prepare(annchor_ctx *c, int32_t n_neighbors, int32_t nmin)
{
    if (!c) return ANNCHOR_EINVAL;
    ANN_REQUIRE(c, c->have_RA, ANNCHOR_EINVAL, "RefineApprox not initialised");
    ANN_REQUIRE(c, n_neighbors >= 1 && nmin >= 0, ANNCHOR_EINVAL, "bad selection parameters");
    ANN_CHECK_HIP(c, hipSetDevice(c->device));
    ANN_TRY(select_stage_a(c, n_neighbors, nmin));
    c->sel_prepared = true; c->sel_k = n_neighbors; c->sel_nmin = nmin;
    return ANNCHOR_OK;
}

extern "C" int annchor_select_candidates(annchor_ctx *c, int32_t n_neighbors, int32_t nmin, const double *errs,
                                         const int64_t *err_ptr, int32_t nlabels, int64_t n_refine, int32_t lookahead,
                                         int64_t *n_cand, int64_t *n_next)
{
    if (!c || (errs && !err_ptr) || !n_cand || !n_next) return ANNCHOR_EINVAL;
    ANN_REQUIRE(c, c->have_RA, ANNCHOR_EINVAL, "RefineApprox not initialised");
    const bool dev_errs = errs == nullptr;
    ANN_REQUIRE(c, !dev_errs || (c->errs_on_device && nlabels == c->model_nb), ANNCHOR_ESTATE,
                "no device-resident residual lists for %d labels (annchor_fit_errors_device)", nlabels);
    ANN_REQUIRE(c, nlabels >= 1 && nlabels <= 255, ANNCHOR_ELIMIT, "1..255 error labels supported");
    ANN_REQUIRE(c, n_neighbors >= 1 && lookahead >= 1 && n_refine >= 0, ANNCHOR_EINVAL, "bad selection parameters");
    if (!dev_errs)
        for (int b = 0; b < nlabels; ++b)
            ANN_REQUIRE(c, err_ptr[b + 1] > err_ptr[b], ANNCHOR_ESTATE, "error bin %d has no samples", b);
    ANN_CHECK_HIP(c, hipSetDevice(c->device));
    const int64_t n = c->n, nx = c->nx;
    if (!(c->sel_prepared && c->sel_k == n_neighbors && c->sel_nmin == nmin)) ANN_TRY(select_stage_a(c, n_neighbors, nmin));
    c->sel_prepared = false;
    ANN_TRY(select_stage_finish(c));
    (void)nx;
    const int64_t nerr = dev_errs ? 2 * c->nsamp + 64 : err_ptr[nlabels];
    if (!dev_errs) {
        ANN_TRY(ann_reserve(c, c->errs, sizeof(double) * (size_t)nerr));
        ANN_TRY(ann_reserve(c, c->errptr, sizeof(int64_t) * (size_t)(MAXBINS > nlabels ? MAXBINS + 1 : nlabels + 1)));
        ANN_TRY(ann_h2d(c, c->errs.p, errs, sizeof(double) * (size_t)nerr));
        ANN_TRY(ann_h2d(c, c->errptr.p, err_ptr, sizeof(int64_t) * (size_t)(nlabels + 1)));
        c->errs_on_device = false; c->model_cache_valid = false;
    }
    {
        const int64_t lds_entries = dev_errs ? c->nsamp + 64 : nerr;
        const int in_lds = lds_entries * 8 <= 60 * 1024;
        const size_t dyn = in_lds ? (size_t)lds_entries * 8 : 0;
        int blocks = min(ann_blocks(n, 256 * 8), c->prop.multiProcessorCount * 8);
        ProfScope ps(c, "ecdf_probability", (double)n * 26.0);
        static const long long index_min = getenv("ANNCHOR_ECDF_INDEX_MIN") ? atoll(getenv("ANNCHOR_ECDF_INDEX_MIN")) : (4ll << 20);
        EcdfIndex *index = nullptr;
        uint32_t *table = nullptr;
        if (n >= index_min && nlabels > 0 && nerr > 0 && nerr < (1ll << 29)) {
            const size_t idx_bytes = (sizeof(EcdfIndex) * (size_t)nlabels + 15) & ~(size_t)15;
            ANN_TRY(ann_reserve(c, c->ecdf_index, idx_bytes + sizeof(uint32_t) * (size_t)(2 * nerr + nlabels + 1)));
            index = c->ecdf_index.as<EcdfIndex>();
            table = reinterpret_cast<uint32_t *>(c->ecdf_index.as<char>() + idx_bytes);
            k_ecdf_index<<<nlabels, 256, 0, c->stream>>>(c->errs.as<double>(), c->errptr.as<int64_t>(), index, table);
        }
        k_prob<<<blocks, 256, dyn, c->stream>>>(n, c->ij.as<int2>(), c->thresh.as<double>(), c->RA.as<double>(),
                                               c->ncm.as<uint8_t>(), c->label.as<uint8_t>(), c->errs.as<double>(),
                                               c->errptr.as<int64_t>(), nlabels, in_lds ? (int)lds_entries : 0, c->prob.as<double>(), n >= ANN_STREAM_MIN_PAIRS,
                                               index, table);
    }
    ANN_CHECK_HIP(c, hipGetLastError());
    int64_t n_unc = 0;
    ANN_TRY(annchor_count_uncomputed(c, &n_unc));
    CutState cs;
    memset(&cs, 0, sizeof cs);
    cs.K1 = n_refine;
    cs.K5 = n_refine * (int64_t)lookahead;
    cs.all1 = n_refine >= n_unc;
    cs.all5 = cs.all1 || cs.K5 >= n_unc;
    cs.t1 = cs.t5 = INFINITY;
    const unsigned long long *d_cut_prefix = nullptr;
    const int *d_cut_unfinished = nullptr;
    int64_t cut_ks[2];
    int cut_nk = 0;
    auto cut_values_waiting = [&]() -> int {
        double tv[2];
        ANN_TRY(ann_kth_smallest(c, c->prob.as<double>(), c->ncm.as<uint8_t>(), n, cut_ks, cut_nk, tv));
        int q = 0;
        if (!cs.all1) cs.t1 = tv[q++];
        if (!cs.all5) cs.t5 = tv[q++];
        return ANNCHOR_OK;
    };
    if (cs.all1) cs.t1 = -1.0;
    if (cs.all5) cs.t5 = -1.0;
    if (n_refine == 0) { cs.all1 = cs.all5 = 0; cs.t1 = cs.t5 = INFINITY; cs.K1 = cs.K5 = 0; }
    const int nsub = cp_nsub(n);
    const int nb = ann_blocks(n, (int64_t)CP_SUBTILE * nsub);
    ANN_TRY(ann_reserve(c, c->sel_state, SEL_STATE_BYTES));
    ANN_TRY(ann_reserve(c, c->blk_cnt, sizeof(uint32_t) * 4 * (size_t)nb));
    ANN_TRY(ann_reserve(c, c->blk_off, sizeof(int64_t) * 4 * (size_t)nb));
    const int64_t maxc = cs.all1 ? n_unc : cs.K1, maxn = cs.all5 ? n_unc : cs.K5;
    ANN_TRY(ann_reserve(c, c->cand, sizeof(int32_t) * (size_t)(maxc + 1)));
    ANN_TRY(ann_reserve(c, c->next, sizeof(int32_t) * (size_t)(maxn + 1)));
    cs.rk1 = cs.rk5 = ~0ull;
    if (n_refine > 0 && !(cs.all1 && cs.all5)) {
        if (!cs.all1) cut_ks[cut_nk++] = n_unc - cs.K1;
        if (!cs.all5) cut_ks[cut_nk++] = n_unc - cs.K5;
        if (!getenv("ANNCHOR_CUT_WAIT")) {
            Sel2Epilogue ep;
            memset(&ep, 0, sizeof ep);
            ep.kind = 2; ep.cs = c->sel_state.as<CutState>(); ep.cs_init = cs; ep.need1 = !cs.all1; ep.need5 = !cs.all5;
            ep.force_redo = getenv("ANNCHOR_CUT_FORCE_REDO") ? 1 : 0;
            ANN_TRY(ann_kth_async(c, c->prob.as<double>(), c->ncm.as<uint8_t>(), n, cut_ks, cut_nk, &d_cut_prefix, &d_cut_unfinished, &ep));
        }
        if (!d_cut_prefix) ANN_TRY(cut_values_waiting());
    }
    const CutState cs_in = cs;
    if (!d_cut_prefix) ANN_TRY(ann_h2d(c, c->sel_state.p, &cs, sizeof cs));
    const bool ties = n_refine > 0 && !(cs.all1 && cs.all5);
    ANN_TRY(ann_reserve(c, c->tie_lists, sizeof(unsigned long long) * 2 * TIE_CAP));
    unsigned long long *tl1 = c->tie_lists.as<unsigned long long>(), *tl5 = tl1 + TIE_CAP;
    auto split = [&]() {
        ProfScope ps(c, "topk_split_compact", (double)n * 16.0 + (double)(maxc + maxn) * 4.0);
        k_cut_count<<<nb, CP_THREADS, 0, c->stream>>>(c->prob.as<double>(), c->RA.as<double>(), n, c->sel_state.as<CutState>(),
                                                     c->blk_cnt.as<uint32_t>(), nsub);
        k_cut_scan<<<1, CS_THREADS, 0, c->stream>>>(c->blk_cnt.as<uint32_t>(), nb, c->sel_state.as<CutState>(), c->blk_off.as<int64_t>());
        k_cut_emit<<<nb, CP_THREADS, 0, c->stream>>>(c->prob.as<double>(), c->RA.as<double>(), n, c->sel_state.as<CutState>(),
                                                    c->blk_off.as<int64_t>(), c->cand.as<int32_t>(), c->next.as<int32_t>(), nsub);
    };
    auto tie_groups = [&]() -> int {
        ProfScope ps(c, "topk_tie_groups", (double)n * 8.0);
        const int tb = (int)std::min<int64_t>(ann_blocks(n, 256 * TIE_U), (int64_t)c->prop.multiProcessorCount * 3);
        const char *cap_env = getenv("ANNCHOR_TIE_CAP");
        const long long cap = cap_env ? std::min<long long>(TIE_CAP, std::max<long long>(1, atoll(cap_env))) : TIE_CAP;
        ANN_TRY(ann_reserve(c, c->tie_hist, sizeof(uint32_t) * 2 * TIE_BINS));
        if (c->tie_hist_clean != c->tie_hist.p) {
            ANN_CHECK_HIP(c, hipMemsetAsync(c->tie_hist.p, 0, sizeof(uint32_t) * 2 * TIE_BINS, c->stream));
            c->tie_hist_clean = c->tie_hist.p;
        }
        k_tie_hist<<<tb, 256, 0, c->stream>>>(c->prob.as<double>(), n, c->sel_state.as<CutState>(), c->tie_hist.as<uint32_t>());
        k_tie_pick<<<1, 1024, 0, c->stream>>>(c->sel_state.as<CutState>(), c->tie_hist.as<uint32_t>());
        k_tie_collect<<<tb, 256, 0, c->stream>>>(c->prob.as<double>(), n, c->sel_state.as<CutState>(), tl1, tl5, cap);
        k_tie_select<<<1, 1024, 0, c->stream>>>(c->sel_state.as<CutState>(), tl1, tl5, cap);
        return ANNCHOR_OK;
    };
    if (ties) ANN_TRY(tie_groups());
    split();
    ANN_CHECK_HIP(c, hipEventRecord(c->call_b, c->stream));
    c->call_timed = true;
    ANN_CHECK_HIP(c, hipGetLastError());
    if (nmin > 0) {
        unsigned char both[SEL_ERR_OFF + 4];
        ANN_TRY(ann_d2h(c, both, c->sel_state.p, sizeof both));
        int32_t e = 0;
        memcpy(&cs, both, sizeof cs);
        memcpy(&e, both + SEL_ERR_OFF, 4);
        c->gn_err_clean = e == 0;
        ANN_REQUIRE(c, e == 0, ANNCHOR_ESTATE, "guarantee_nmin: a row has fewer not-computed candidates than it must refine");
    } else {
        ANN_TRY(ann_d2h(c, &cs, c->sel_state.p, sizeof cs));
    }
    if (d_cut_prefix) {
        ann_kth_async_done(c);
        if (cs.sel_unfinished) {
            cs = cs_in;
            ANN_TRY(cut_values_waiting());
            ANN_TRY(ann_h2d(c, c->sel_state.p, &cs, sizeof cs));
            if (ties) ANN_TRY(tie_groups());
            split();
            ANN_CHECK_HIP(c, hipGetLastError());
            ANN_TRY(ann_d2h(c, &cs, c->sel_state.p, sizeof cs));
        }
    }
    if (cs.tie_overflow) {
        ANN_TRY(ann_reserve(c, c->marked, (size_t)n));
        for (int q = 0; q < 2; ++q) {
            const bool all = q == 0 ? cs.all1 : cs.all5;
            const int64_t cnt = q == 0 ? cs.tie_n1 : cs.tie_n5, e = q == 0 ? cs.K1 - cs.tie_gt1 : cs.K5 - cs.tie_gt5;
            unsigned long long rk = ~0ull;
            if (!all && e < cnt) {
                if (e <= 0) rk = 0ull;
                else {
                    ANN_TRY(ann_reserve(c, c->colT, sizeof(double) * (size_t)n));
                    k_tie_flags<<<ann_blocks(n, 256), 256, 0, c->stream>>>(c->prob.as<double>(), n, q == 0 ? cs.t1 : cs.t5, c->marked.as<uint8_t>(),
                                                                          c->colT.as<double>());
                    int64_t kq = e - 1;
                    double rv = 0;
                    ANN_TRY(ann_kth_smallest(c, c->colT.as<double>(), c->marked.as<uint8_t>(), n, &kq, 1, &rv));
                    rk = (unsigned long long)rv;
                }
            }
            if (q == 0) cs.rk1 = rk; else cs.rk5 = rk;
        }
        cs.tie_overflow = 0; cs.e1 = cs.e5 = 0; cs.ncand = cs.nnext = 0;
        ANN_TRY(ann_h2d(c, c->sel_state.p, &cs, sizeof cs));
        split();
        ANN_CHECK_HIP(c, hipGetLastError());
        ANN_TRY(ann_d2h(c, &cs, c->sel_state.p, sizeof cs));
    }
    c->ncand = cs.ncand;
    c->n_unc = n_unc;
    c->cand_marked = false;
    c->nnext = cs.nnext;
    *n_cand = cs.ncand;
    *n_next = cs.nnext;
    return ANNCHOR_OK;
}

__global__ void k_mark_candidates(const int32_t *__restrict__ pos, int64_t m, uint8_t *__restrict__ ncm)
{
    int64_t t = (int64_t)blockIdx.x * blockDim.x + threadIdx.x;
    if (t < m) ncm[pos[t]] = 0;
}

extern "C" int annchor_mark_candidates(annchor_ctx *c)
{
    if (!c) return ANNCHOR_EINVAL;
    ANN_REQUIRE(c, c->have_RA, ANNCHOR_EINVAL, "RefineApprox not initialised");
    if (c->ncand == 0 || c->cand_marked) return ANNCHOR_OK;
    ANN_CHECK_HIP(c, hipSetDevice(c->device));
    k_mark_candidates<<<ann_blocks(c->ncand, 256), 256, 0, c->stream>>>(c->cand.as<int32_t>(), c->ncand, c->ncm.as<uint8_t>());
    ANN_CHECK_HIP(c, hipGetLastError());
    if (c->n_unc >= 0) c->n_unc -= c->ncand;
    c->cand_marked = true; c->sel_prepared = false;
    return ANNCHOR_OK;
}

extern "C" int annchor_park_refine(annchor_ctx *c, int32_t action)
{
    if (!c || (action != 1 && action != 2)) return ANNCHOR_EINVAL;
    if (action == 1) { c->park_refine = true; return ANNCHOR_OK; }
    if (!c->park_refine) return ANNCHOR_OK;
    c->park_refine = false;
    return annchor_refine_candidates(c);
}

extern "C" int annchor_refine_candidates(annchor_ctx *c)
{
    if (!c) return ANNCHOR_EINVAL;
    ANN_REQUIRE(c, c->have_RA, ANNCHOR_EINVAL, "RefineApprox not initialised");
    ANN_REQUIRE(c, c->metric != ANNCHOR_METRIC_NONE, ANNCHOR_EINVAL, "no device metric bound to this context");
    if (c->ncand == 0) return ANNCHOR_OK;
    ANN_CHECK_HIP(c, hipSetDevice(c->device));
    PairSource src;
    src.ij = c->ij.as<int2>();
    src.idx = c->cand.as<int32_t>();
    src.n = c->ncand;
    ANN_CHECK_HIP(c, hipEventRecord(c->call_a, c->stream));
    ANN_TRY(ann_metric_launch(c, src, nullptr, c->RA.as<double>(), c->ncm.as<uint8_t>()));
    ANN_CHECK_HIP(c, hipEventRecord(c->call_b, c->stream));
    c->call_timed = true;
    ANN_CHECK_HIP(c, hipGetLastError());
    if (c->n_unc >= 0 && !c->cand_marked) c->n_unc -= c->ncand;
    c->cand_marked = true; c->sel_prepared = false;
    return ANNCHOR_OK;
}

__global__ void k_write_refined(const int32_t *__restrict__ pos, const double *__restrict__ v, int64_t m,
                                double *__restrict__ RA, uint8_t *__restrict__ ncm)
{
    int64_t t = (int64_t)blockIdx.x * blockDim.x + threadIdx.x;
    if (t < m) { RA[pos[t]] = v[t]; ncm[pos[t]] = 0; }
}

extern "C" int annchor_set_refined(annchor_ctx *c, const double *exact, int64_t n_cand)
{
    if (!c || (n_cand > 0 && !exact)) return ANNCHOR_EINVAL;
    ANN_REQUIRE(c, c->have_RA, ANNCHOR_EINVAL, "RefineApprox not initialised");
    ANN_REQUIRE(c, n_cand == c->ncand, ANNCHOR_EINVAL, "expected %lld refined values, got %lld", (long long)c->ncand,
                (long long)n_cand);
    if (n_cand == 0) return ANNCHOR_OK;
    ANN_CHECK_HIP(c, hipSetDevice(c->device));
    ANN_TRY(ann_reserve(c, c->stage_in, sizeof(double) * (size_t)n_cand));
    ANN_TRY(ann_h2d(c, c->stage_in.p, exact, sizeof(double) * (size_t)n_cand));
    k_write_refined<<<ann_blocks(n_cand, 256), 256, 0, c->stream>>>(c->cand.as<int32_t>(), c->stage_in.as<double>(), n_cand,
                                                                   c->RA.as<double>(), c->ncm.as<uint8_t>());
    ANN_CHECK_HIP(c, hipGetLastError());
    if (c->n_unc >= 0 && !c->cand_marked) c->n_unc -= n_cand;
    c->cand_marked = true; c->sel_prepared = false;
    return ANNCHOR_OK;
}
```

annchor_amd/csrc/selstate.h:

```cpp
#pragma once
#include "common.h"

struct BinEdges {
    double e[MAXBINS + 1];
    int nb;
};

struct SamplerStats {
    BinEdges be;
    double q[2];
    unsigned long long counts[MAXBINS];
    int unfinished;
};

struct CutState {
    double t1, t5;
    int64_t K1, K5;
    int64_t e1, e5;
    int64_t ncand, nnext;
    int all1, all5;
    unsigned long long rk1, rk5;
    int64_t tie_n1, tie_n5;
    int64_t tie_gt1, tie_gt5;
    long long tie_bin1, tie_bin5;
    long long tie_rem1, tie_rem5;
    long long tie_len1, tie_len5;
    int64_t tie_got1, tie_got5;
    int tie_overflow;
    int sel_unfinished;
};

struct Sel2Epilogue {
    int kind;
    SamplerStats *st;
    int nparts;
    CutState *cs;
    CutState cs_init;
    int need1, need5, force_redo;
};

__device__ __forceinline__ void sel2_epilogue(const Sel2Epilogue &ep, const uint64_t *prefix , int unfinished)
{
    if (ep.kind == 1) {
        SamplerStats *st = ep.st;
        const int nparts = ep.nparts;
        const double q1 = ann_key_asc_inv(prefix[0]), q3 = ann_key_asc_inv(prefix[1]);
        st->q[0] = q1; st->q[1] = q3;
        const int num = nparts - 1, div = num > 1 ? num - 1 : 1;
        const double delta = q3 - q1, step = delta / (double)div;
        st->be.nb = nparts;
        st->be.e[0] = -INFINITY;
        for (int i = 0; i < num; ++i) {
            double y;
            if (step != 0.0) { const double p = (double)i * step; y = p + q1; }
            else { const double p = ((double)i / (double)div) * delta; y = p + q1; }
            if (num > 1 && i == num - 1) y = q3;
            st->be.e[1 + i] = y;
        }
        st->be.e[nparts] = INFINITY;
        for (int b = 0; b < MAXBINS; ++b) st->counts[b] = 0;
        st->unfinished = unfinished;
    } else if (ep.kind == 2) {
        CutState init = ep.cs_init;
        int q = 0;
        if (ep.need1) init.t1 = ann_key_asc_inv(prefix[q++]);
        if (ep.need5) init.t5 = ann_key_asc_inv(prefix[q++]);
        init.sel_unfinished = unfinished | ep.force_redo;
        *ep.cs = init;
    }
}
```

include/annchor_hip.h:

```cpp
#ifndef ANNCHOR_HIP_H
#define ANNCHOR_HIP_H

#include <stdint.h>

#ifdef __cplusplus
extern "C" {
#endif

typedef struct annchor_ctx annchor_ctx;

enum {
    ANNCHOR_OK = 0,
    ANNCHOR_EINVAL = -1,
    ANNCHOR_EHIP = -2,
    ANNCHOR_ENODEV = -3,
    ANNCHOR_ELIMIT = -4,
    ANNCHOR_ESTATE = -5
};

enum { ANNCHOR_METRIC_NONE = 0, ANNCHOR_METRIC_LEVENSHTEIN = 1, ANNCHOR_METRIC_EUCLIDEAN_F32 = 2,
       ANNCHOR_METRIC_EUCLIDEAN_F64 = 3, ANNCHOR_METRIC_WASSERSTEIN = 4, ANNCHOR_METRIC_COSINE_F32 = 5,
       ANNCHOR_METRIC_COSINE_F64 = 6 };

enum {
// ... 59 lines not shown
int annchor_bin_counts(annchor_ctx *ctx, const double *bins, int32_t nbins, int64_t *counts);
int annchor_sampler_stats(annchor_ctx *ctx, const int64_t *ks, int32_t n_partitions, double *q, double *edges, int64_t *counts,
                          int32_t *fused);
int annchor_select_by_rank(annchor_ctx *ctx, const double *bins, int32_t nbins, const int32_t *bin_of,
                           const int64_t *ranks, int64_t nreq, int64_t *positions);
int annchor_legacy_prefetch(uint32_t seed, int64_t ndraws);
int annchor_legacy_generate(uint32_t seed, int64_t ndraws);
int annchor_legacy_generate_at_next_wait(annchor_ctx *ctx, uint32_t seed, int64_t ndraws, int64_t chunk);
int annchor_legacy_choice_ranks(uint32_t seed, const int64_t *counts, const int64_t *want, int32_t nbins,
                                int64_t *ranks_out, int64_t *n_out);
int annchor_legacy_choice_begin(uint32_t seed, const int64_t *counts, const int64_t *want, int32_t nbins, void **ticket);
int annchor_legacy_choice_end(void *ticket, int64_t *ranks_out, int64_t *n_out);

int annchor_ols_bins(void *dgelsd_ptr, const double *X, const double *y, int64_t ld, int32_t nf, const int64_t *cuts,
                     int32_t nbins, double *coef, double *xmean, double *ymean, int32_t *status);
int annchor_gather_features(annchor_ctx *ctx, const int64_t *pos, int64_t m, double *feats);
int annchor_evaluate_samples(annchor_ctx *ctx, const int64_t *pos, int64_t m, double *sample_y);
int annchor_sample_pairs(annchor_ctx *ctx, const double *bins, int32_t nbins, const int64_t *counts, const int32_t *bin_of,
                         const int64_t *ranks, int64_t nreq, int64_t *positions, double *feats, double *sample_y);
int annchor_set_samples(annchor_ctx *ctx, const int64_t *pos, int64_t m, const double *sample_y);

int annchor_predict_merge(annchor_ctx *ctx, const double *bins, int32_t nb, const double *W,
                          const double *c, int32_t first_iteration, int32_t is_metric,
                          double *sample_predict);
int annchor_merge_host_prediction(annchor_ctx *ctx, const double *pred, int32_t first_iteration,
                                  int32_t is_metric);
int annchor_set_labels(annchor_ctx *ctx, const int64_t *labels);

int annchor_sample_pairs_device(annchor_ctx *ctx, const double *bins, int32_t nbins, const int64_t *counts, const int32_t *bin_of,
                                const int64_t *ranks, int64_t nreq);
int annchor_hash_sample_pairs_device(annchor_ctx *ctx, const double *bins, int32_t nbins, const int64_t *counts, const int64_t *want,
                                     uint64_t seed_key, int64_t *n_out);
int annchor_sample_pairs_device_draw(annchor_ctx *ctx, const double *bins, int32_t nbins, const int64_t *counts, const int64_t *want,
                                     uint32_t seed, int64_t *n_out, int32_t *taken);
int annchor_legacy_choice_ranks_device(annchor_ctx *ctx, uint32_t seed, const int64_t *counts, const int64_t *want, int32_t nbins,
                                       int64_t *ranks_out, int32_t *taken);
int annchor_download_samples(annchor_ctx *ctx, int64_t *positions, double *feats, double *sample_y, double *sample_predict);
int annchor_fit_regression_device(annchor_ctx *ctx, const double *bins, int32_t nbins, int32_t first_iteration, int32_t is_metric);
int annchor_fit_errors_device(annchor_ctx *ctx);
int annchor_model_download(annchor_ctx *ctx, double *W, double *c, int32_t *status, int64_t *err_ptr, int32_t *flags );
int annchor_errors_download(annchor_ctx *ctx, double *errs, int64_t n_errs);
int annchor_model_download_with_errors(annchor_ctx *ctx, double *W, double *c, int32_t *status, int64_t *err_ptr, int32_t *flags ,
                                       double *errs, int64_t errs_cap, int64_t *n_errs);

int annchor_select_candidates(annchor_ctx *ctx, int32_t n_neighbors, int32_t nmin, const double *errs,
                              const int64_t *err_ptr, int32_t nlabels, int64_t n_refine,
                              int32_t lookahead, int64_t *n_cand, int64_t *n_next);
int annchor_select_prepare(annchor_ctx *ctx, int32_t n_neighbors, int32_t nmin);
int annchor_mark_candidates(annchor_ctx *ctx);
int annchor_refine_candidates(annchor_ctx *ctx);
int annchor_lev_persist_state(int set);

int annchor_park_refine(annchor_ctx *ctx, int32_t action);
int annchor_set_refined(annchor_ctx *ctx, const double *exact, int64_t n_cand);

int annchor_update_bounds(annchor_ctx *ctx);

int annchor_neighbor_graph(annchor_ctx *ctx, int32_t n_neighbors, int64_t *ng_idx, double *ng_dist);

int annchor_stream_bind(annchor_ctx *ctx, const float *X, int64_t n_local, int32_t dim, int64_t global_base,
                        int32_t x_on_device);
int annchor_stream_anchor_round(annchor_ctx *ctx, const float *anchor_vec, int32_t round, int32_t n_anchors,
                                double *local_max, int64_t *local_arg);
int annchor_stream_get_row(annchor_ctx *ctx, int64_t local_idx, float *out);
int annchor_stream_order(annchor_ctx *ctx, int32_t min_tiles, void **Xs, void **rs, void **perm, void **lo, void **hi,
                         void **mid, int64_t *n_pad, int32_t *n_tiles, int32_t *dim_padded);
int annchor_stream_order_begin(annchor_ctx *ctx, int32_t min_tiles, int32_t tile_begin, int32_t tile_count, void **order_local,
                               void **order_all, int64_t *order_bytes);
int annchor_stream_order_end(annchor_ctx *ctx, void **Xs, void **rs, void **perm, void **lo, void **hi, void **mid, int64_t *n_pad,
                             int32_t *n_tiles, int32_t *dim_padded);
int annchor_stream_knn(annchor_ctx *ctx, const void *Xs_all, const void *rs_all, const void *perm_all, const void *lo_all,
                       const void *hi_all, const void *mid_all, int64_t n_all, int32_t nt_all, int32_t n_anchors, int32_t dim_padded,
                       int32_t tile_begin, int32_t tile_count, int32_t k, double p_work, int32_t join_passes, int32_t join_extra,
                       int64_t *row_ids, int64_t *ng_idx, double *ng_dist, int64_t *tile_evals);
int annchor_stream_knn_run(annchor_ctx *ctx, const void *Xs_all, const void *rs_all, const void *perm_all, const void *lo_all,
                           const void *hi_all, const void *mid_all, int64_t n_all, int32_t nt_all, int32_t n_anchors,
                           int32_t dim_padded, int32_t tile_begin, int32_t tile_count, int32_t k, double p_work, int32_t join_passes,
                           int32_t join_extra, int64_t *tile_evals);
int annchor_stream_knn_fetch(annchor_ctx *ctx, int64_t *row_ids, int64_t *ng_idx, double *ng_dist);
int annchor_stream_knn_begin(annchor_ctx *ctx, const void *Xs_all, const void *rs_all, const void *perm_all, const void *lo_all,
                             const void *hi_all, const void *mid_all, int64_t n_all, int32_t nt_all, int32_t n_anchors,
                             int32_t dim_padded, int32_t tile_begin, int32_t tile_count, int32_t k, int32_t tile_budget,
                             void **lists_local, int64_t *lists_bytes);
int annchor_stream_knn_join(annchor_ctx *ctx, const void *lists_all, int32_t per_pass, void **lists_local, int64_t *updates);
int annchor_stream_join_rev_begin(annchor_ctx *ctx, const void *lists_all, void **rev_local, void **rev_all, int64_t *rev_bytes);
int annchor_stream_budget(int32_t n_tiles, double p_work, int32_t join_passes, int32_t *total, int32_t *tile_phase,
                          int32_t *per_pass);
int annchor_stream_knn_end(annchor_ctx *ctx, int64_t *row_ids, int64_t *ng_idx, double *ng_dist, int64_t *tile_evals);
int annchor_stream_last_counts(annchor_ctx *ctx, int64_t *tile_phase_evals, int64_t *join_chunks);
int annchor_stream_last_kernel(annchor_ctx *ctx, int32_t *kind, int64_t *guard_rows);
int annchor_stream_last_tile_kernels(annchor_ctx *ctx, int32_t *two_stage, int32_t *repaired);
int annchor_stream_query(annchor_ctx *ctx, const void *Xs_all, const void *rs_all, const void *perm_all, const void *lo_all,
                         const void *hi_all, const void *mid_all, int64_t n_all, int32_t nt_all, int32_t n_anchors, int32_t dim_padded,
                         int32_t nn, double p_work, int64_t *out_idx, double *out_dist, int64_t *tile_evals);
int annchor_stream_bind_f64(annchor_ctx *ctx, const double *X, int64_t n_local, int32_t dim, int64_t global_base, const double *centre_in,
                            double *centre_out, void **rows64);
int annchor_stream_rerank64(annchor_ctx *ctx, int32_t k, int64_t *ng_idx, double *ng_dist);
int annchor_stream_query64(annchor_ctx *ctx, const void *Xs_all, const void *rs_all, const void *perm_all, const void *lo_all,
                           const void *hi_all, const void *mid_all, int64_t n_all, int32_t nt_all, int32_t n_anchors, int32_t dim_padded,
                           int32_t nn, int32_t nn_search, double p_work, const void *rows64_data, int64_t n_data, int64_t data_base,
                           int64_t *out_idx, double *out_dist, int64_t *tile_evals);
int annchor_stream_last_rerank64(annchor_ctx *ctx, int64_t *flagged_rows, int32_t *repaired);
int annchor_stream_order_classes(annchor_ctx *ctx, const int32_t *labels, int32_t n_classes, const float *anchor_vecs, int64_t *n_pad,
                                 int32_t *n_tiles, int32_t *dim_padded);
int annchor_stream_enemies(annchor_ctx *ctx, int32_t nn, double p_work, int64_t *out_idx, double *out_dist, int64_t *tile_evals);
int annchor_stream_join_tables(annchor_ctx *ctx, const void *gathered, int32_t world, int32_t n_anchors, int32_t n_tiles,
// ... 62 lines not shown
```

Measured before the change: 364.5 graphs/s.

## Chain candidate selection into refinement speculatively with device-side go flag

Candidate selection no longer blocks on a host readback of the cut state and graph-neighbor error flags. It predicts the candidate counts, seals the result in a device report, and launches the mark and Levenshtein refinement kernels gated by a device 'go' flag. The host checks the report later and falls back to resuming the selection synchronously if the prediction was wrong. This removes a host-device synchronization per iteration, at the cost of extra state, possibly wasted or redone work on mispredictions, and added complexity.

```diff
diff --git a/annchor_amd/_native.py b/annchor_amd/_native.py
--- a/annchor_amd/_native.py
+++ b/annchor_amd/_native.py
@@ -83,6 +83,9 @@
     "annchor_mark_candidates": (ctypes.c_int, [_vp]),
     "annchor_refine_candidates": (ctypes.c_int, [_vp]),
     "annchor_park_refine": (ctypes.c_int, [_vp, _i32]),
+    "annchor_chain_request": (ctypes.c_int, [_vp, _i32, _i32]),
+    "annchor_chain_check": (ctypes.c_int, [_vp, ctypes.POINTER(_i32), ctypes.POINTER(_i64)]),
+    "annchor_select_resume": (ctypes.c_int, [_vp, ctypes.POINTER(_i64), ctypes.POINTER(_i64)]),
     "annchor_set_refined": (ctypes.c_int, [_vp, _vp, _i64]),
     "annchor_update_bounds": (ctypes.c_int, [_vp]),
     "annchor_neighbor_graph": (ctypes.c_int, [_vp, _i32, _vp, _vp]),
@@ -680,6 +683,19 @@
     def park_refine(self, action):
         self._chk(self.lib.annchor_park_refine(self.h, int(action)))
 
+    def chain_request(self, on, gn_batch=0):
+        self._chk(self.lib.annchor_chain_request(self.h, int(bool(on)), int(gn_batch)))
+
+    def chain_check(self):
+        st, cnt = _i32(), (_i64 * 2)()
+        self._chk(self.lib.annchor_chain_check(self.h, ctypes.byref(st), cnt))
+        return st.value, (cnt[0], cnt[1])
+
+    def select_resume(self):
+        nc, nn = _i64(), _i64()
+        self._chk(self.lib.annchor_select_resume(self.h, ctypes.byref(nc), ctypes.byref(nn)))
+        return nc.value, nn.value
+
     def set_refined(self, exact):
         exact = _c(exact, np.float64)
         self._chk(self.lib.annchor_set_refined(self.h, _ptr(exact), len(exact)))
diff --git a/annchor_amd/annchor.py b/annchor_amd/annchor.py
--- a/annchor_amd/annchor.py
+++ b/annchor_amd/annchor.py
@@ -454,6 +454,8 @@
         self._pair_list_stage("fit_predict_errors")
         if self._pipelined and self._fit_it is not None:
             nn = self.n_neighbors
+            if self._device_metric:
+                self._engine.chain_request(True, self.__dict__.get("_gn_batch", 0))
             self._engine.select_prepare(nn, 3 * nn // 2 if self._fit_it == 0 else 0)
         if self.__dict__.get("_model_on_device"):
             self._engine.fit_errors_device()
@@ -498,6 +500,25 @@
             ncand, nnext = self._engine.select_candidates(nn, nmin, errs, n_refine, self.lookahead)
         self.n_refine = n_refine
         self._invalidate("RA", "thresh", "cand", "next")
+        self._queue_refinement(ncand, it)
+        if self._pipelined and it < self.niters - 1:
+            ncand, _ = self._settle_chain(ncand, it)
+        else:
+            self._chain_open = (ncand, it) if self._pipelined else None
+        self.evals += ncand
+        self._invalidate("RA", "ncm")
+
+    def _settle_chain(self, ncand, it):
+        status, _ = self._engine.chain_check()
+        if not status:
+            return ncand, False
+        self._sample_ticket = None
+        ncand, _ = self._engine.select_resume()
+        self._invalidate("RA", "thresh", "cand", "next")
+        self._queue_refinement(ncand, it)
+        return ncand, True
+
+    def _queue_refinement(self, ncand, it):
         if self._pipelined and self._device_metric and ncand and it < self.niters - 1 and self._sampler_on_device():
             self._engine.mark_candidates()
             self._engine.park_refine(1)
@@ -512,8 +533,6 @@
             mapback = self._engine.download(_native.F_CAND)
             exact = np.asarray(self.get_exact_ijs(self.f, self.X, self.IJs[mapback]), dtype=np.float64)
             self._engine.set_refined(exact)
-        self.evals += ncand
-        self._invalidate("RA", "ncm")
 
     def _adopt_device_model(self, nb):
         W, c, status, ep, flags, flat = self._engine.model_download_with_errors(nb, 2 * int(self.n_samples) + 16)
@@ -549,6 +568,14 @@
     def get_ann(self):
         self._pair_list_stage("get_ann")
         self.neighbor_graph = self._engine.neighbor_graph(self.n_neighbors)
+        open_, self._chain_open = self.__dict__.get("_chain_open"), None
+        if open_ is not None:
+            expected, it = open_
+            ncand, redone = self._settle_chain(expected, it)
+            if redone:
+                self._invalidate("RA", "ncm")
+                self.neighbor_graph = self._engine.neighbor_graph(self.n_neighbors)
+            self.evals += ncand - expected
 
     def fit(self):
         if self._streamed is not None:
@@ -600,6 +627,7 @@
         finally:
             self._pipelined, self._fit_it, self._sample_ticket = False, None, None
             self._make_stream = None
+            self._engine.chain_request(False)
 
     def _fit_stages(self, stage, make_stream, t, origin):
         stage("get_anchors", self.get_anchors)
diff --git a/annchor_amd/csrc/common.h b/annchor_amd/csrc/common.h
--- a/annchor_amd/csrc/common.h
+++ b/annchor_amd/csrc/common.h
@@ -138,7 +138,17 @@
     bool sel_prepared = false;
     int sel_k = 0, sel_nmin = 0;
     bool gn_pending = false;
-    int gn_round = 0, gn_L = 0;
+    int gn_round = 0, gn_L = 0, gn_nb = 0;
+    bool chain_req = false;
+    int chain_gn_batch = 0;
+    bool chain_stage_a = false;
+    bool chain_pending = false;
+    bool chain_waited = false;
+    bool chain_failed = false;
+    int32_t chain_why = 0;
+    int64_t chain_fallbacks = 0;
+    int64_t chain_runs = 0;
+    struct { int32_t nmin, nlabels, lookahead; int64_t n_refine, nerr, lds_entries; } chain_args = {};
     DevBuf sel_hist, sel_state, blk_cnt, blk_off;
     DevBuf sel_pass_state;
     DevBuf tie_lists, tie_hist;
@@ -282,6 +292,7 @@
     const int32_t *idx = nullptr;
     const int32_t *anchor = nullptr;
     int64_t n = 0;
+    const int32_t *go = nullptr;
     const double *pick_row = nullptr;
     double *pick_runmin = nullptr;
     int32_t *pick_out = nullptr;
diff --git a/annchor_amd/csrc/ctx.hip b/annchor_amd/csrc/ctx.hip
--- a/annchor_amd/csrc/ctx.hip
+++ b/annchor_amd/csrc/ctx.hip
@@ -219,6 +219,7 @@
     const long long t_w = timing ? ann_now_ns() : 0;
     const hipError_t rc = c->comm ? ann_comm_guarded_sync(c, c->stream, where) : hipStreamSynchronize(c->stream);
     if (timing) fprintf(stderr, "T wait %s %lld %lld %lld\n", where, t_in, t_w, ann_now_ns());
+    c->chain_waited = true;
     if (c->lev_ap_probe_epoch) ann_lev_ap_probe(c);
     return rc;
 }
@@ -280,6 +281,7 @@
     if (trace) fprintf(stderr, "sync %s\n", __func__);
     const long long t_w = timing ? ann_now_ns() : 0;
     ANN_CHECK_HIP(c, hipEventSynchronize(c->dl_ev));
+    c->chain_waited = true;
     if (timing) fprintf(stderr, "T wait %s %lld %lld %lld\n", __func__, t_w, t_w, ann_now_ns());
     memcpy(dst, slot, bytes);
     return rc;
diff --git a/annchor_amd/csrc/lev.hip b/annchor_amd/csrc/lev.hip
--- a/annchor_amd/csrc/lev.hip
+++ b/annchor_amd/csrc/lev.hip
@@ -49,6 +49,7 @@
     const int32_t *perm;
     const int32_t *n0;
     int GL0, P0;
+    const int32_t *go;
 };
 
 #define LEVR_PAD 64
@@ -248,6 +249,7 @@
     a.text_stride = 2 * (2 * LEVR_PAD + ((c->maxlen + 15) & ~15) + 16);
     a.wave_bytes = a.pm_bytes + a.P * a.text_stride + 256;
     ar.b = a;
+    ar.go = nullptr;
     ar.pick_row = nullptr; ar.pick_runmin = nullptr; ar.pick_out = nullptr; ar.pick_reset = 0; ar.pick_nx = 0;
     if (src.anchor && src.pick_fused && c->nx <= 8192) {
         *src.pick_fused = true;
@@ -285,6 +287,7 @@
 {
     extern __shared__ __attribute__((aligned(16))) unsigned char smem[];
     const LevArgs &a = ar.b;
+    if (ar.go && *ar.go == 0) return;
     const int lane = threadIdx.x;
     const int A = a.alphabet;
     unsigned char *pm_col = smem + (size_t)(lane >> 5) * A * LEVF_ROW + (size_t)(lane & 31) * 4;
@@ -445,9 +448,10 @@
 __global__ __launch_bounds__(256) void k_lev_classify(const int2 *__restrict__ ij, const int32_t *__restrict__ idx,
                                                       const int32_t *__restrict__ slen, int64_t n, int gl0,
                                                       int32_t *__restrict__ perm, int32_t *__restrict__ cursors,
-                                                      int32_t *__restrict__ next_cursors)
+                                                      int32_t *__restrict__ next_cursors, const int32_t *go)
 {
     if (blockIdx.x == 0 && threadIdx.x < 2) next_cursors[threadIdx.x] = 0;
+    if (go && *go == 0) return;
     __shared__ int wcnt[2][4];
     __shared__ int base[2];
     const int lane = threadIdx.x & 63, wave = threadIdx.x >> 6;
@@ -514,12 +518,13 @@
             int32_t *cursors = nullptr, *next_cursors = nullptr;
             ANN_TRY(lev_next_cursors(c, &cursors, &next_cursors));
             k_lev_classify<<<ann_blocks(npairs, 256), 256, 0, c->stream>>>(src.ij, src.idx, a.slen, npairs, c->lev_gl0, perm,
-                                                                           cursors, next_cursors);
+                                                                           cursors, next_cursors, src.go);
             ar.perm = perm; ar.n0 = cursors; ar.GL0 = c->lev_gl0; ar.P0 = P0;
         }
     }
     a.wave_bytes = a.pm_bytes + (ar.perm ? ar.P0 : a.P) * a.text_stride + 256;
     ar.b = a;
+    ar.go = src.go;
     ar.pick_row = nullptr; ar.pick_runmin = nullptr; ar.pick_out = nullptr; ar.pick_reset = 0; ar.pick_nx = 0;
     if (src.anchor && src.pick_fused && c->nx <= 8192) {
         *src.pick_fused = true;
@@ -760,12 +765,14 @@
     double *RA;
     uint8_t *ncm;
     int alphabet, pm_bytes, fb_stride, buf_stride, pad;
+    const int32_t *go;
 };
 
 __global__ __launch_bounds__(ANN_WAVE) void k_lev_p2(LevArgsP2 aa)
 {
     extern __shared__ __attribute__((aligned(16))) unsigned char smem[];
     const LevArgsP2 &a = aa;
+    if (a.go && *a.go == 0) return;
     const int lane = threadIdx.x, A = a.alphabet;
     const int n_short = a.cursors[0], n_long = a.cursors[1];
     const int ws = (n_short + 1) >> 1;
@@ -1222,6 +1229,7 @@
     LevArgsP2 a;
     a.sym = c->sym.as<uint8_t>(); a.soff = c->soff.as<int32_t>(); a.slen = c->slen.as<int32_t>();
     a.ij = src.ij; a.idx = src.idx; a.n = src.n; a.out = d_out; a.RA = d_RA; a.ncm = d_ncm;
+    a.go = src.go;
     a.alphabet = c->alphabet;
     a.pm_bytes = 2 * a.alphabet * LEVF_ROW;
     a.fb_stride = (c->maxlen + 2 + 7) & ~7;
@@ -1234,7 +1242,7 @@
     int32_t *perm = c->lev_perm.as<int32_t>();
     int32_t *cursors = nullptr, *next_cursors = nullptr;
     ANN_TRY(lev_next_cursors(c, &cursors, &next_cursors));
-    k_lev_classify<<<ann_blocks(src.n, 256), 256, 0, c->stream>>>(src.ij, src.idx, a.slen, src.n, 16, perm, cursors, next_cursors);
+    k_lev_classify<<<ann_blocks(src.n, 256), 256, 0, c->stream>>>(src.ij, src.idx, a.slen, src.n, 16, perm, cursors, next_cursors, src.go);
     a.perm = perm; a.cursors = cursors;
     if (lds > 64 * 1024)
         ANN_CHECK_HIP(c, hipFuncSetAttribute((const void *)k_lev_p2, hipFuncAttributeMaxDynamicSharedMemorySize, (int)lds));
@@ -1552,6 +1560,8 @@
 int ann_lev_launch(annchor_ctx *c, const PairSource &src, double *d_out, double *d_RA, uint8_t *d_ncm)
 {
     if (src.n == 0) return ANNCHOR_OK;
+    ANN_REQUIRE(c, !src.go || (!c->sym_wide && !src.anchor && (c->maxlen + 31) / 32 <= 32), ANNCHOR_ESTATE,
+                "chained refinement on a kernel that does not read its flag");
     if (c->sym_wide) return launch_w(c, src, d_out, d_RA, d_ncm);
     LevArgs a;
     a.sym = c->sym.as<uint8_t>();
diff --git a/annchor_amd/csrc/select.hip b/annchor_amd/csrc/select.hip
--- a/annchor_amd/csrc/select.hip
+++ b/annchor_amd/csrc/select.hip
@@ -152,8 +152,10 @@
                                                  const int32_t *__restrict__ gl_cnt, const int32_t *__restrict__ gl_ncomp,
                                                  const uint32_t *__restrict__ cur, uint32_t *__restrict__ nxt,
                                                  const int32_t *__restrict__ mout_cur, int32_t *__restrict__ mout_nxt,
-                                                 int32_t *__restrict__ mout_clr, int32_t *__restrict__ changed, int32_t *__restrict__ err)
-{
+                                                 int32_t *__restrict__ mout_clr, int32_t *__restrict__ changed, int32_t *__restrict__ err,
+                                                 const int32_t *prev_changed)
+{
+    if (prev_changed && *prev_changed == 0) return;
     const int lane = threadIdx.x & 63;
     const int64_t i = ((int64_t)blockIdx.x * blockDim.x + threadIdx.x) >> 6;
     if (i >= nx) return;
@@ -223,9 +225,11 @@
 }
 
 __global__ void k_gn_apply(int64_t nx, int L, int Lw, const int32_t *__restrict__ gl_pos, const int32_t *__restrict__ gl_cnt,
-                           const uint32_t *__restrict__ masks, double *__restrict__ RA)
+                           const uint32_t *__restrict__ masks, double *__restrict__ RA, const int32_t *last_changed,
+                           int32_t *unsettled)
 {
     const int64_t t = (int64_t)blockIdx.x * blockDim.x + threadIdx.x;
+    if (last_changed && *last_changed != 0) { if (t == 0) *unsettled = 1; return; }
     if (t >= nx * L) return;
     const int64_t i = t / L;
     const int e = (int)(t - i * L);
@@ -891,7 +895,7 @@
 #define CS_THREADS 1024
 #define CS_ITEMS 4
 __global__ __launch_bounds__(CS_THREADS) void k_cut_scan(const uint32_t *__restrict__ blk, int nb, CutState *__restrict__ cs,
-                                                        int64_t *__restrict__ off)
+                                                        int64_t *__restrict__ off, ChainSeal seal)
 {
     __shared__ unsigned long long wsum[CS_THREADS / 64];
     const int lane = threadIdx.x & 63, wave = threadIdx.x >> 6;
@@ -965,7 +969,17 @@
             exo += outv[e];
         }
     }
-    if (threadIdx.x == 0) { cs->e1 = e1; cs->e5 = e5; cs->ncand = (int64_t)(c_out & 0xffffffffull); cs->nnext = (int64_t)(c_out >> 32); }
+    if (threadIdx.x == 0) {
+        const int64_t ncand = (int64_t)(c_out & 0xffffffffull), nnext = (int64_t)(c_out >> 32);
+        cs->e1 = e1; cs->e5 = e5; cs->ncand = ncand; cs->nnext = nnext;
+        if (seal.rep) {
+            int32_t why = (ncand != seal.exp_cand || nnext != seal.exp_next) ? 1 : 0;
+            if (cs->sel_unfinished) why |= 2;
+            if (cs->tie_overflow) why |= 4;
+            if (seal.gn_flags) { if (seal.gn_flags[1]) why |= 8; if (seal.gn_flags[0]) why |= 16; }
+            seal.rep->go = why == 0; seal.rep->why = why; seal.rep->ncand = ncand; seal.rep->nnext = nnext;
+        }
+    }
 }
 
 __global__ __launch_bounds__(CP_THREADS) void k_cut_emit(const double *__restrict__ prob, const double *__restrict__ RA, int64_t n,
@@ -1037,9 +1051,25 @@
 }
 
 #define SEL_ERR_OFF 256
+#define SEL_CHAIN_OFF (SEL_ERR_OFF + 16)
 #define SEL_STATE_BYTES (SEL_ERR_OFF + 256)
 static_assert(sizeof(CutState) <= SEL_ERR_OFF, "the error flag sits behind the cut state");
 static inline int32_t *gn_err_ptr(annchor_ctx *c) { return reinterpret_cast<int32_t *>(c->sel_state.as<char>() + SEL_ERR_OFF); }
+static inline ChainReport *chain_report_ptr(annchor_ctx *c) { return reinterpret_cast<ChainReport *>(c->sel_state.as<char>() + SEL_CHAIN_OFF); }
+static_assert(SEL_CHAIN_OFF + sizeof(ChainReport) <= SEL_STATE_BYTES && sizeof(ChainReport) + 16 <= annchor_ctx::PIN_TAIL_BYTES, "report layout");
+static inline unsigned char *chain_report_host(annchor_ctx *c)
+{
+    return c->pin + (size_t)annchor_ctx::PIN_SLOTS * annchor_ctx::PIN_SLOT_BYTES + annchor_ctx::PIN_DL_BYTES + 16;
+}
+static bool chain_eligible(annchor_ctx *c)
+{
+    if (!c->chain_req || !c->pin) return false;
+    const char *e = getenv("ANNCHOR_CHAIN_REFINE");
+    if (e && atoi(e) == 0) return false;
+    if (getenv("ANNCHOR_CUT_WAIT")) return false;
+    const char *er = getenv("ANNCHOR_LEV_R");
+    return c->metric == ANNCHOR_METRIC_LEVENSHTEIN && !c->sym_wide && (c->maxlen + 31) / 32 <= 32 && !(er && atoi(er) == 1);
+}
 size_t ann_sel_state_bytes() { return SEL_STATE_BYTES; }
 #define GN_BATCH 8
 
@@ -1068,7 +1098,7 @@
         ANN_TRY(ann_reserve(c, c->gl_ncomp, sizeof(int32_t) * (size_t)nx));
         ANN_TRY(ann_reserve(c, c->sel_state, SEL_STATE_BYTES));
         if (!c->gn_err_clean) {
-            ANN_CHECK_HIP(c, hipMemsetAsync(gn_err_ptr(c), 0, 4, c->stream));
+            ANN_CHECK_HIP(c, hipMemsetAsync(gn_err_ptr(c), 0, 8, c->stream));
         }
         c->gn_err_clean = false;
         {
@@ -1099,13 +1129,15 @@
             for (int q = 0; q < 3; ++q) mout[q] = reinterpret_cast<int32_t *>(c->gn_state.as<char>() + 2 * mask_bytes + q * mout_bytes);
             int32_t *changed = reinterpret_cast<int32_t *>(c->gn_state.as<char>() + 2 * mask_bytes + 3 * mout_bytes);
             ANN_CHECK_HIP(c, hipMemsetAsync(c->gn_state.p, 0, 2 * mask_bytes + 3 * mout_bytes + sizeof(int32_t) * GN_BATCH, c->stream));
+            c->chain_stage_a = chain_eligible(c);
+            const int gnb = c->chain_stage_a && c->chain_gn_batch > 0 ? std::min(c->chain_gn_batch, GN_BATCH) : GN_BATCH;
             int round = 0;
-            for (int q = 0; q < GN_BATCH; ++q, ++round)
+            for (int q = 0; q < gnb; ++q, ++round)
                 k_gn_round<<<ann_blocks(nx * 64, 256), 256, 0, c->stream>>>(
                     nx, nmin, L, Lw, c->gl_val.as<double>(), oth, twin, c->gl_cnt.as<int32_t>(), c->gl_ncomp.as<int32_t>(),
                     masks[round & 1], masks[(round + 1) & 1], mout[round % 3], mout[(round + 1) % 3], mout[(round + 2) % 3],
-                    changed + q, gn_err_ptr(c));
-            c->gn_pending = true; c->gn_round = round; c->gn_L = L;
+                    changed + q, gn_err_ptr(c), c->chain_stage_a && q > 0 ? changed + q - 1 : nullptr);
+            c->gn_pending = true; c->gn_round = round; c->gn_L = L; c->gn_nb = gnb;
         } else if (L <= GN_LMAX && ring_lds <= 156 * 1024) {
             ProfScope ps(c, "guarantee_nmin_sweep", (double)nx * L * 21.0);
             int32_t *oth = c->gl_pos.as<int32_t>() + (size_t)nx * L, *twin = oth + (size_t)nx * L;
@@ -1142,7 +1174,7 @@
     return ANNCHOR_OK;
 }
 
-static int select_stage_finish(annchor_ctx *c)
+static int select_stage_finish(annchor_ctx *c, bool chained = false)
 {
     if (!c->gn_pending) return ANNCHOR_OK;
     const int64_t nx = c->nx;
@@ -1154,20 +1186,28 @@
     int32_t *changed = reinterpret_cast<int32_t *>(c->gn_state.as<char>() + 2 * mask_bytes + 3 * mout_bytes);
     int32_t *oth = c->gl_pos.as<int32_t>() + (size_t)nx * L, *twin = oth + (size_t)nx * L;
     int round = c->gn_round;
+    const int gnb = c->gn_nb > 0 ? c->gn_nb : GN_BATCH;
+    if (chained) {
+        k_gn_apply<<<ann_blocks(nx * L, 256), 256, 0, c->stream>>>(nx, L, Lw, c->gl_pos.as<int32_t>(), c->gl_cnt.as<int32_t>(),
+                                                                  masks[round & 1], c->RA.as<double>(), changed + gnb - 1,
+                                                                  gn_err_ptr(c) + 1);
+        ANN_CHECK_HIP(c, hipGetLastError());
+        return ANNCHOR_OK;
+    }
     for (;;) {
         int32_t h_changed[GN_BATCH];
         ANN_TRY(ann_d2h(c, h_changed, changed, sizeof h_changed));
-        if (h_changed[GN_BATCH - 1] == 0) break;
+        if (h_changed[gnb - 1] == 0) break;
         ANN_REQUIRE(c, round <= (int)nx + GN_BATCH, ANNCHOR_EHIP, "guarantee_nmin rounds did not settle");
         ANN_CHECK_HIP(c, hipMemsetAsync(changed, 0, sizeof(int32_t) * GN_BATCH, c->stream));
-        for (int q = 0; q < GN_BATCH; ++q, ++round)
+        for (int q = 0; q < gnb; ++q, ++round)
             k_gn_round<<<ann_blocks(nx * 64, 256), 256, 0, c->stream>>>(
                 nx, nmin, L, Lw, c->gl_val.as<double>(), oth, twin, c->gl_cnt.as<int32_t>(), c->gl_ncomp.as<int32_t>(),
                 masks[round & 1], masks[(round + 1) & 1], mout[round % 3], mout[(round + 1) % 3], mout[(round + 2) % 3],
-                changed + q, gn_err_ptr(c));
+                changed + q, gn_err_ptr(c), c->chain_stage_a && q > 0 ? changed + q - 1 : nullptr);
     }
     k_gn_apply<<<ann_blocks(nx * L, 256), 256, 0, c->stream>>>(nx, L, Lw, c->gl_pos.as<int32_t>(), c->gl_cnt.as<int32_t>(),
-                                                              masks[round & 1], c->RA.as<double>());
+                                                              masks[round & 1], c->RA.as<double>(), nullptr, nullptr);
     ANN_CHECK_HIP(c, hipGetLastError());
     c->gn_pending = false;
     return ANNCHOR_OK;
@@ -1185,6 +1225,9 @@
     c->sel_prepared = true; c->sel_k = n_neighbors; c->sel_nmin = nmin;
     return ANNCHOR_OK;
 }
+
+static int select_tail(annchor_ctx *c, int32_t nmin, int32_t nlabels, int64_t nerr, int64_t lds_entries, int64_t n_refine,
+                       int32_t lookahead, bool chained, int64_t *n_cand, int64_t *n_next);
 
 extern "C" int annchor_select_candidates(annchor_ctx *c, int32_t n_neighbors, int32_t nmin, const double *errs,
                                          const int64_t *err_ptr, int32_t nlabels, int64_t n_refine, int32_t lookahead,
@@ -1204,8 +1247,10 @@
     const int64_t n = c->n, nx = c->nx;
     if (!(c->sel_prepared && c->sel_k == n_neighbors && c->sel_nmin == nmin)) ANN_TRY(select_stage_a(c, n_neighbors, nmin));
     c->sel_prepared = false;
-    ANN_TRY(select_stage_finish(c));
     (void)nx;
+    const bool chained = chain_eligible(c) && (!c->gn_pending || c->chain_stage_a);
+    c->chain_pending = c->chain_failed = false;
+    ANN_TRY(select_stage_finish(c, chained));
     const int64_t nerr = dev_errs ? 2 * c->nsamp + 64 : err_ptr[nlabels];
     if (!dev_errs) {
         ANN_TRY(ann_reserve(c, c->errs, sizeof(double) * (size_t)nerr));
@@ -1214,8 +1259,16 @@
         ANN_TRY(ann_h2d(c, c->errptr.p, err_ptr, sizeof(int64_t) * (size_t)(nlabels + 1)));
         c->errs_on_device = false; c->model_cache_valid = false;
     }
+    const int64_t lds_entries = dev_errs ? c->nsamp + 64 : nerr;
+    c->chain_args = {nmin, nlabels, lookahead, n_refine, nerr, lds_entries};
+    return select_tail(c, nmin, nlabels, nerr, lds_entries, n_refine, lookahead, chained, n_cand, n_next);
+}
+
+static int select_tail(annchor_ctx *c, int32_t nmin, int32_t nlabels, int64_t nerr, int64_t lds_entries, int64_t n_refine,
+                       int32_t lookahead, bool chained, int64_t *n_cand, int64_t *n_next)
+{
+    const int64_t n = c->n;
     {
-        const int64_t lds_entries = dev_errs ? c->nsamp + 64 : nerr;
         const int in_lds = lds_entries * 8 <= 60 * 1024;
         const size_t dyn = in_lds ? (size_t)lds_entries * 8 : 0;
         int blocks = min(ann_blocks(n, 256 * 8), c->prop.multiProcessorCount * 8);
@@ -1286,11 +1339,19 @@
     const bool ties = n_refine > 0 && !(cs.all1 && cs.all5);
     ANN_TRY(ann_reserve(c, c->tie_lists, sizeof(unsigned long long) * 2 * TIE_CAP));
     unsigned long long *tl1 = c->tie_lists.as<unsigned long long>(), *tl5 = tl1 + TIE_CAP;
+    ChainSeal seal;
+    memset(&seal, 0, sizeof seal);
+    if (chained) {
+        seal.exp_cand = n_refine == 0 ? 0 : (cs.all1 ? n_unc : cs.K1);
+        seal.exp_next = n_refine == 0 ? 0 : (cs.all1 && cs.all5 ? n_unc : (cs.all5 ? n_unc : cs.K5) - seal.exp_cand);
+        seal.gn_flags = nmin > 0 ? gn_err_ptr(c) : nullptr;
+        seal.rep = chain_report_ptr(c);
+    }
     auto split = [&]() {
         ProfScope ps(c, "topk_split_compact", (double)n * 16.0 + (double)(maxc + maxn) * 4.0);
         k_cut_count<<<nb, CP_THREADS, 0, c->stream>>>(c->prob.as<double>(), c->RA.as<double>(), n, c->sel_state.as<CutState>(),
                                                      c->blk_cnt.as<uint32_t>(), nsub);
-        k_cut_scan<<<1, CS_THREADS, 0, c->stream>>>(c->blk_cnt.as<uint32_t>(), nb, c->sel_state.as<CutState>(), c->blk_off.as<int64_t>());
+        k_cut_scan<<<1, CS_THREADS, 0, c->stream>>>(c->blk_cnt.as<uint32_t>(), nb, c->sel_state.as<CutState>(), c->blk_off.as<int64_t>(), seal);
         k_cut_emit<<<nb, CP_THREADS, 0, c->stream>>>(c->prob.as<double>(), c->RA.as<double>(), n, c->sel_state.as<CutState>(),
                                                     c->blk_off.as<int64_t>(), c->cand.as<int32_t>(), c->next.as<int32_t>(), nsub);
     };
@@ -1315,6 +1376,18 @@
     ANN_CHECK_HIP(c, hipEventRecord(c->call_b, c->stream));
     c->call_timed = true;
     ANN_CHECK_HIP(c, hipGetLastError());
+    if (chained) {
+        ANN_CHECK_HIP(c, hipMemcpyAsync(chain_report_host(c), seal.rep, sizeof(ChainReport), hipMemcpyDeviceToHost, c->stream));
+        c->chain_pending = true; c->chain_waited = false;
+        ++c->chain_runs;
+        if (d_cut_prefix) ann_kth_async_done(c);
+        c->ncand = seal.exp_cand; c->nnext = seal.exp_next;
+        c->n_unc = n_unc;
+        c->cand_marked = false;
+        *n_cand = c->ncand; *n_next = c->nnext;
+        return ANNCHOR_OK;
+    }
+    seal.rep = nullptr;
     if (nmin > 0) {
         unsigned char both[SEL_ERR_OFF + 4];
         ANN_TRY(ann_d2h(c, both, c->sel_state.p, sizeof both));
@@ -1373,11 +1446,13 @@
     return ANNCHOR_OK;
 }
 
-__global__ void k_mark_candidates(const int32_t *__restrict__ pos, int64_t m, uint8_t *__restrict__ ncm)
-{
+__global__ void k_mark_candidates(const int32_t *__restrict__ pos, int64_t m, uint8_t *__restrict__ ncm, const int32_t *go)
+{
+    if (go && *go == 0) return;
     int64_t t = (int64_t)blockIdx.x * blockDim.x + threadIdx.x;
     if (t < m) ncm[pos[t]] = 0;
 }
+static inline const int32_t *chain_go(annchor_ctx *c) { return c->chain_pending ? &chain_report_ptr(c)->go : nullptr; }
 
 extern "C" int annchor_mark_candidates(annchor_ctx *c)
 {
@@ -1385,7 +1460,7 @@
     ANN_REQUIRE(c, c->have_RA, ANNCHOR_EINVAL, "RefineApprox not initialised");
     if (c->ncand == 0 || c->cand_marked) return ANNCHOR_OK;
     ANN_CHECK_HIP(c, hipSetDevice(c->device));
-    k_mark_candidates<<<ann_blocks(c->ncand, 256), 256, 0, c->stream>>>(c->cand.as<int32_t>(), c->ncand, c->ncm.as<uint8_t>());
+    k_mark_candidates<<<ann_blocks(c->ncand, 256), 256, 0, c->stream>>>(c->cand.as<int32_t>(), c->ncand, c->ncm.as<uint8_t>(), chain_go(c));
     ANN_CHECK_HIP(c, hipGetLastError());
     if (c->n_unc >= 0) c->n_unc -= c->ncand;
     c->cand_marked = true; c->sel_prepared = false;
@@ -1412,6 +1487,7 @@
     src.ij = c->ij.as<int2>();
     src.idx = c->cand.as<int32_t>();
     src.n = c->ncand;
+    src.go = chain_go(c);
     ANN_CHECK_HIP(c, hipEventRecord(c->call_a, c->stream));
     ANN_TRY(ann_metric_launch(c, src, nullptr, c->RA.as<double>(), c->ncm.as<uint8_t>()));
     ANN_CHECK_HIP(c, hipEventRecord(c->call_b, c->stream));
@@ -1446,3 +1522,52 @@
     c->cand_marked = true; c->sel_prepared = false;
     return ANNCHOR_OK;
 }
+
+extern "C" int annchor_chain_request(annchor_ctx *c, int32_t on, int32_t gn_batch)
+{
+    if (!c || gn_batch < 0) return ANNCHOR_EINVAL;
+    c->chain_req = on != 0;
+    c->chain_gn_batch = gn_batch;
+    return ANNCHOR_OK;
+}
+
+extern "C" int annchor_chain_check(annchor_ctx *c, int32_t *status, int64_t *counts)
+{
+    if (!c || !status) return ANNCHOR_EINVAL;
+    *status = 0;
+    if (counts) { counts[0] = c->chain_fallbacks; counts[1] = c->chain_runs; }
+    if (!c->chain_pending) return ANNCHOR_OK;
+    ANN_CHECK_HIP(c, hipSetDevice(c->device));
+    if (!c->chain_waited) ANN_CHECK_HIP(c, ann_sync(c, __func__));
+    ChainReport rep;
+    memcpy(&rep, chain_report_host(c), sizeof rep);
+    c->chain_pending = false;
+    if (rep.go) {
+        if (c->chain_args.nmin > 0) c->gn_err_clean = true;
+        c->gn_pending = false;
+        return ANNCHOR_OK;
+    }
+    if (c->cand_marked && c->n_unc >= 0) c->n_unc += c->ncand;
+    c->cand_marked = false;
+    c->ncand = c->nnext = 0;
+    c->chain_failed = true; c->chain_why = rep.why;
+    ++c->chain_fallbacks;
+    if (counts) counts[0] = c->chain_fallbacks;
+    *status = rep.why ? rep.why : 1;
+    return ANNCHOR_OK;
+}
+
+extern "C" int annchor_select_resume(annchor_ctx *c, int64_t *n_cand, int64_t *n_next)
+{
+    if (!c || !n_cand || !n_next) return ANNCHOR_EINVAL;
+    ANN_REQUIRE(c, c->chain_failed, ANNCHOR_ESTATE, "no chained selection to resume");
+    ANN_CHECK_HIP(c, hipSetDevice(c->device));
+    c->chain_failed = false;
+    if (c->chain_why & 8) {
+        ANN_CHECK_HIP(c, hipMemsetAsync(gn_err_ptr(c) + 1, 0, 4, c->stream));
+        ANN_TRY(select_stage_finish(c, false));
+    }
+    c->gn_pending = false;
+    const auto &a = c->chain_args;
+    return select_tail(c, a.nmin, a.nlabels, a.nerr, a.lds_entries, a.n_refine, a.lookahead, false, n_cand, n_next);
+}
diff --git a/annchor_amd/csrc/selstate.h b/annchor_amd/csrc/selstate.h
--- a/annchor_amd/csrc/selstate.h
+++ b/annchor_amd/csrc/selstate.h
@@ -28,6 +28,16 @@
     int64_t tie_got1, tie_got5;
     int tie_overflow;
     int sel_unfinished;
+};
+
+struct ChainReport {
+    int32_t go, why;
+    int64_t ncand, nnext;
+};
+struct ChainSeal {
+    int64_t exp_cand, exp_next;
+    const int32_t *gn_flags;
+    ChainReport *rep;
 };
 
 struct Sel2Epilogue {
diff --git a/include/annchor_hip.h b/include/annchor_hip.h
--- a/include/annchor_hip.h
+++ b/include/annchor_hip.h
@@ -135,6 +135,9 @@
 int annchor_lev_persist_state(int set);
 
 int annchor_park_refine(annchor_ctx *ctx, int32_t action);
+int annchor_chain_request(annchor_ctx *ctx, int32_t on, int32_t gn_batch);
+int annchor_chain_check(annchor_ctx *ctx, int32_t *status, int64_t *counts);
+int annchor_select_resume(annchor_ctx *ctx, int64_t *n_cand, int64_t *n_next);
 int annchor_set_refined(annchor_ctx *ctx, const double *exact, int64_t n_cand);
 
 int annchor_update_bounds(annchor_ctx *ctx);
```

Result: slower. 336.0 graphs/s (-7.8%).
